# AY-Liu/Image-Editing-Framework

Hardware: AMD Instinct MI355X
Metric: denoising steps/sec (SD1.5 512x512 P2P edit step, UNet batch 4) (higher is better)
Workload: dtype f16x3; 1 GPU; sd15 UNet (859.5M params) P2P AttentionRefine edit step, 2 prompts x CFG = batch 4, 64x64 latents (512x512 px), 50-step DDIM, guidance 7.5, cross 0.8 / self 0.4, per-step null-text unconditional embeddings (P2P_NTI, edit_real.py); one independent edit per GPU; precision mode f16x3: fp32 storage; every contraction on split operands: hi + lo fp16 halves of each fp32 element, Ah Bh + Al Bh + Ah Bl =

## Files before the change

image-editing-framework_amd/csrc/exact_f32.hip:

```cpp
#include "ief_common.h"
#include "ief_params.h"
#include "x3_common.h"

#define XBM 128
#define XBK 32
#define XLD 36

__device__ __forceinline__ float silu_x(float x) { return x / (1.0f + expf(-x)); }

struct RowCoord { int b, oy, ox, ok; };

template <bool CONV, bool TRANSB, int NT>
__global__ __launch_bounds__(256) void igemm_f32_kernel(const IefGemmF32Params p) {
    constexpr int XBN = 64 * NT;
    __shared__ __attribute__((aligned(16))) float smem_x[2 * (XBM + XBN) * XLD];
    float* As = smem_x;
    float* Bs = smem_x + 2 * XBM * XLD;
    const int tid = threadIdx.x, lane = tid & 63, wid = tid >> 6;
    const int wm = wid >> 1, wn = wid & 1;
    const int li = lane & 31, lh = lane >> 5;
    const int ntn = (p.N + XBN - 1) / XBN;
    const int tm = blockIdx.x / ntn, tn = blockIdx.x - tm * ntn;
    const int m0 = tm * XBM, n0 = tn * XBN;
    const float* A = p.A;
// ... 875 lines not shown
static inline void gn3b_chunks(int HW, int C, int* nch, int* P) {
    const int CQ = C >> 2, CQB = CQ < 256 ? CQ : 256, PY = 256 / CQB;
    int p = GN3B_U * PY;
    if (p > HW) p = HW;
    *P = p;
    *nch = (HW + p - 1) / p;
}
extern "C" long long ief_groupnorm_bwd_f32_ws_floats(int B, int HW, int C) {
    int nch, P;
    gn3b_chunks(HW, C, &nch, &P);
    return ief_groupnorm_f32_ws_floats(B, HW, C) + 2ll * B * nch * C + 4ll * B * C;
}
__device__ __forceinline__ float dsilu_z(float z) {
    const float sg = 1.0f / (1.0f + expf(-z));
    return sg * (1.0f + z * (1.0f - sg));
}
template <int MODE>
__global__ __launch_bounds__(256) void gn3_bwd_kernel(const float* __restrict__ x, const float* __restrict__ x2, int C1, int C2,
                                                      const float* __restrict__ dy, const float* __restrict__ add, int HW, int P,
                                                      const float* __restrict__ gstats, const float* __restrict__ mom, int groups,
                                                      const float* __restrict__ gamma, const float* __restrict__ beta, int silu,
                                                      float* __restrict__ p1, float* __restrict__ p2, float* __restrict__ dx,
                                                      float* __restrict__ dx2) {
    __shared__ f32x4 red[256];
    const int C = C1 + C2, CQ = C >> 2, cpg = C / groups;
    const int CQB = CQ < 256 ? CQ : 256, PY = 256 / CQB;
    const int tid = threadIdx.x, cq = tid % CQB, py = tid / CQB;
    const bool lane_ok = py < PY;
    const int chunk = blockIdx.x, b = blockIdx.y, nch = gridDim.x;
    const int p0 = chunk * P, pn = min(P, HW - p0);
    for (int qb = 0; qb * CQB < CQ; ++qb) {
        const int q = qb * CQB + cq;
        const bool ok = lane_ok && q < CQ;
        const int c = ok ? q * 4 : 0;
        int cs = 4;
        const float* src = gn3_src(x, x2, C1, C2, b, HW, c, &cs) + (long long)p0 * cs;
        const float* dsrc = dy + ((long long)b * HW + p0) * C + c;
        f32x4 mu, rs, m1 = {0.f, 0.f, 0.f, 0.f}, m2 = {0.f, 0.f, 0.f, 0.f};
#pragma unroll
        for (int j = 0; j < 4; ++j) {
            const int g = (c + j) / cpg;
            mu[j] = gstats[((long long)b * groups + g) * 2];
            rs[j] = gstats[((long long)b * groups + g) * 2 + 1];
            if (MODE == 1) { m1[j] = mom[((long long)b * groups + g) * 2]; m2[j] = mom[((long long)b * groups + g) * 2 + 1]; }
        }
        const f32x4 ga = *(const f32x4*)(gamma + c), be = *(const f32x4*)(beta + c);
        f32x4 v[GN3B_U], d[GN3B_U];
#pragma unroll
        for (int u = 0; u < GN3B_U; ++u) {
            const int pp = py + u * PY;
            const bool in = ok && pp < pn;
            v[u] = in ? *(const f32x4*)(src + (long long)pp * cs) : f32x4{0.f, 0.f, 0.f, 0.f};
            d[u] = in ? *(const f32x4*)(dsrc + (long long)pp * C) : f32x4{0.f, 0.f, 0.f, 0.f};
        }
        f32x4 s1 = {0.f, 0.f, 0.f, 0.f}, s2 = {0.f, 0.f, 0.f, 0.f};
#pragma unroll
        for (int u = 0; u < GN3B_U; ++u) {
            const int pp = py + u * PY;
            if (!(ok && pp < pn)) continue;
            const f32x4 xh = (v[u] - mu) * rs;
            f32x4 gv = d[u] * ga;
            if (silu) {
#pragma unroll
                for (int j = 0; j < 4; ++j) gv[j] *= dsilu_z(xh[j] * ga[j] + be[j]);
            }
            if (MODE == 0) { s1 += gv; s2 += gv * xh; }
            else {
                f32x4 r = rs * (gv - m1 - xh * m2);
                if (add) r += *(const f32x4*)(add + ((long long)b * HW + p0 + pp) * C + c);
                float* dst = c < C1 ? dx + ((long long)b * HW + p0 + pp) * C1 + c : dx2 + ((long long)b * HW + p0 + pp) * C2 + (c - C1);
                *(f32x4*)dst = r;
            }
        }
        if (MODE == 0) {
            __syncthreads();
            red[tid] = s1;
            __syncthreads();
            f32x4 t1 = {0.f, 0.f, 0.f, 0.f};
            if (ok && py == 0) for (int y = 0; y < PY; ++y) t1 += red[y * CQB + cq];
            __syncthreads();
            red[tid] = s2;
            __syncthreads();
            if (ok && py == 0) {
                f32x4 t2 = {0.f, 0.f, 0.f, 0.f};
                for (int y = 0; y < PY; ++y) t2 += red[y * CQB + cq];
                const long long o = ((long long)b * nch + chunk) * C + c;
                *(f32x4*)(p1 + o) = t1;
                *(f32x4*)(p2 + o) = t2;
            }
        }
    }
}
__global__ __launch_bounds__(256) void gn3_bwd_finalize_kernel(const float* __restrict__ p1, const float* __restrict__ p2, int C, int HW,
                                                               int nch, int groups, float* __restrict__ mom) {
    __shared__ float sa[4], sb[4];
    const int b = blockIdx.x / groups, g = blockIdx.x - b * groups, cpg = C / groups, tid = threadIdx.x, lane = tid & 63;
    const int cl = tid % cpg, r0 = tid / cpg, rstep = 256 / cpg;
    float a = 0.f, q = 0.f;
    if (r0 < rstep) {
        const float* pa = p1 + (long long)b * nch * C + g * cpg + cl;
        const float* pq = p2 + (long long)b * nch * C + g * cpg + cl;
        for (int ch = r0; ch < nch; ch += rstep) { a += pa[(long long)ch * C]; q += pq[(long long)ch * C]; }
    }
#pragma unroll
    for (int off = 32; off > 0; off >>= 1) { a += __shfl_xor(a, off); q += __shfl_xor(q, off); }
    if (lane == 0) { sa[tid >> 6] = a; sb[tid >> 6] = q; }
    __syncthreads();
    if (tid == 0) {
        const float inv = 1.0f / ((float)HW * (float)cpg);
        mom[(long long)blockIdx.x * 2] = ((sa[0] + sa[1]) + (sa[2] + sa[3])) * inv;
        mom[(long long)blockIdx.x * 2 + 1] = ((sb[0] + sb[1]) + (sb[2] + sb[3])) * inv;
    }
}
extern "C" int ief_groupnorm_bwd_f32_ws(const float* x, const float* x2, int C1, int C2, const float* dy, const float* add, float* dx,
                                        float* dx2, const float* gamma, const float* beta, int B, int HW, int groups, float eps,
                                        int silu, float* ws, long long ws_floats, void* stream) {
    if (!x || !dy || !dx || !gamma || !beta || !ws || (C2 > 0 && (!x2 || !dx2))) return IEF_EINVAL;
    if (B <= 0 || HW <= 0 || groups <= 0 || C1 <= 0 || C2 < 0 || (C1 + C2) % groups || (C1 & 3) || (C2 & 3)) return IEF_ESHAPE;
    const int C = C1 + C2;
    if (C / groups > 256) return IEF_ESHAPE;
    if (ws_floats < ief_groupnorm_bwd_f32_ws_floats(B, HW, C)) return IEF_EINVAL;
    if (((uintptr_t)x | (uintptr_t)dy | (uintptr_t)dx | (uintptr_t)ws | (uintptr_t)(x2 ? x2 : x) | (uintptr_t)(dx2 ? dx2 : dx) |
         (uintptr_t)(add ? add : dy) | (uintptr_t)gamma | (uintptr_t)beta) & 15) return IEF_EALIGN;
    int nch, P, nchb, Pb;
    gn3_chunks(HW, C, &nch, &P);
    gn3b_chunks(HW, C, &nchb, &Pb);
    float* pmean = ws;
    float* pm2 = pmean + (long long)B * nch * C;
    float* scale = pm2 + (long long)B * nch * C;
    float* shift = scale + (long long)B * C;
    float* q1 = shift + (long long)B * C;
    float* q2 = q1 + (long long)B * nchb * C;
    float* gstats = q2 + (long long)B * nchb * C;
    float* mom = gstats + 2ll * B * groups;
    hipStream_t st = (hipStream_t)stream;
    hipLaunchKernelGGL(gn3_stats_kernel, dim3(nch, B), dim3(256), 0, st, x, x2, C1, C2, HW, P, pmean, pm2);
    IEF_LAUNCH_CHECK();
    hipLaunchKernelGGL(gn3_finalize_kernel, dim3(B * groups), dim3(256), 0, st, pmean, pm2, C, HW, P, nch, groups, eps, gamma, beta,
                       scale, shift, gstats);
    IEF_LAUNCH_CHECK();
    hipLaunchKernelGGL(gn3_bwd_kernel<0>, dim3(nchb, B), dim3(256), 0, st, x, x2, C1, C2, dy, add, HW, Pb, gstats, (const float*)nullptr,
                       groups, gamma, beta, silu, q1, q2, dx, dx2);
    IEF_LAUNCH_CHECK();
    hipLaunchKernelGGL(gn3_bwd_finalize_kernel, dim3(B * groups), dim3(256), 0, st, q1, q2, C, HW, nchb, groups, mom);
    IEF_LAUNCH_CHECK();
    hipLaunchKernelGGL(gn3_bwd_kernel<1>, dim3(nchb, B), dim3(256), 0, st, x, x2, C1, C2, dy, add, HW, Pb, gstats, mom, groups, gamma,
                       beta, silu, q1, q2, dx, dx2);
    IEF_LAUNCH_CHECK();
    return IEF_OK;
}

extern "C" int ief_groupnorm_silu_f32(const float* x, const float* x2, int C1, int C2, float* out, const float* gamma,
                                      const float* beta, int B, int HW, int groups, float eps, int silu, void* stream) {
    if (!x || !out || !gamma || !beta || (C2 > 0 && !x2)) return IEF_EINVAL;
    if (B <= 0 || HW <= 0 || groups <= 0 || C1 <= 0 || C2 < 0 || (C1 + C2) % groups) return IEF_ESHAPE;
    const int cpg = (C1 + C2) / groups;
    const bool al8 = (((uintptr_t)x | (uintptr_t)(x2 ? x2 : x) | (uintptr_t)out) & 7) == 0;
    if ((cpg & 1) || (C1 & 1) || (cpg >> 1) > 256 || !al8) {
        hipLaunchKernelGGL(groupnorm_f32_scalar_kernel, dim3(B * groups), dim3(256), 0, (hipStream_t)stream, x, x2, C1, C2, out,
                           gamma, beta, HW, groups, eps, silu);
        IEF_LAUNCH_CHECK();
        return IEF_OK;
    }
    const int cp2 = cpg >> 1;
    int PY = 512 / cp2;
    if (PY > HW) PY = HW;
    int threads = ((cp2 * PY + 63) / 64) * 64;
    if (threads > 512) { PY -= 1; threads = ((cp2 * PY + 63) / 64) * 64; }
    const int rounds = (HW + PY * 8 - 1) / (PY * 8);
    int KS = 1;
    while (KS * 2 <= rounds && B * groups * KS < 1024) KS *= 2;
    hipLaunchKernelGGL(groupnorm_f32_kernel, dim3(B * groups * KS), dim3(threads), 0, (hipStream_t)stream, x, x2, C1, C2, out,
                       gamma, beta, HW, groups, eps, silu, PY, KS);
    IEF_LAUNCH_CHECK();
    return IEF_OK;
}

extern "C" int ief_groupnorm_silu_x3p_small(const float* x, const float* x2, int C1, int C2, ief_half* outp, long long plane,
                                            const float* gamma, const float* beta, int B, int HW, int groups, float eps, int silu,
                                            void* stream) {
    if (!x || !outp || !gamma || !beta || (C2 > 0 && !x2)) return IEF_EINVAL;
    if (B <= 0 || HW <= 0 || groups <= 0 || C1 <= 0 || C2 < 0 || (C1 + C2) % groups || (plane & 1)) return IEF_ESHAPE;
    const int cpg = (C1 + C2) / groups;
    if ((cpg & 1) || (C1 & 1) || (cpg >> 1) > 256) return IEF_ESHAPE;
    if ((((uintptr_t)x | (uintptr_t)(x2 ? x2 : x)) & 7) || ((uintptr_t)outp & 3)) return IEF_EALIGN;
    const int cp2 = cpg >> 1;
    int PY = 512 / cp2;
    if (PY > HW) PY = HW;
    int threads = ((cp2 * PY + 63) / 64) * 64;
    if (threads > 512) { PY -= 1; threads = ((cp2 * PY + 63) / 64) * 64; }
    const int rounds = (HW + PY * 8 - 1) / (PY * 8);
    int KS = 1;
    while (KS * 2 <= rounds && B * groups * KS < 1024) KS *= 2;
    hipLaunchKernelGGL(groupnorm_f32_kernel, dim3(B * groups * KS), dim3(threads), 0, (hipStream_t)stream, x, x2, C1, C2, (float*)nullptr,
                       gamma, beta, HW, groups, eps, silu, PY, KS, (half_t*)outp, plane);
    IEF_LAUNCH_CHECK();
    return IEF_OK;
}

template <int E>
__global__ __launch_bounds__(1024) void groupnorm_reg_kernel(const float* __restrict__ x, const float* __restrict__ x2, int C1, int C2,
                                                             float* __restrict__ out, half_t* __restrict__ outp, long long plane,
                                                             const float* __restrict__ gamma, const float* __restrict__ beta, int HW,
                                                             int groups, float eps, int silu) {
    typedef __attribute__((ext_vector_type(2))) float f32x2;
    __shared__ float red[16];
    __shared__ float bc;
    __shared__ float sc_s[512], sh_s[512];
    const int C = C1 + C2, cpg = C / groups, cp2 = cpg >> 1;
    const int b = blockIdx.x / groups, g = blockIdx.x - b * groups;
    const int npairs = HW * cp2;
    const int tid = threadIdx.x;
    const int dq = 1024 / cp2, dr = 1024 - dq * cp2;
    int p = tid / cp2, j = tid - p * cp2;
    f32x2 v[E];
    const int p00 = p, j00 = j;
    const float* xb = x + (long long)b * HW * C1;
    const float* x2b = x2 ? x2 + (long long)b * HW * C2 : x;
#pragma unroll
    for (int k = 0; k < E; ++k) {
        const bool ok = tid + k * 1024 < npairs;
        const int c = g * cpg + (ok ? 2 * j : 0), pp = ok ? p : 0;
        const float* src = c < C1 ? xb + (unsigned)(pp * C1 + c) : x2b + (unsigned)(pp * C2 + (c - C1));
        const f32x2 t = *(const f32x2*)src;
        v[k] = ok ? t : (f32x2){0.f, 0.f};
        p += dq; j += dr;
        if (j >= cp2) { j -= cp2; ++p; }
        if ((k & 3) == 3) __builtin_amdgcn_sched_barrier(0);
    }
    auto block_sum = [&](float t) -> float {
        t = wave_sum(t);
        __syncthreads();
        if ((tid & 63) == 0) red[tid >> 6] = t;
        __syncthreads();
        if (tid == 0) { float a = 0.f; for (int w = 0; w < 16; ++w) a += red[w]; bc = a; }
        __syncthreads();
        return bc;
    };
    float s = 0.f;
#pragma unroll
    for (int k = 0; k < E; ++k) s += v[k][0] + v[k][1];
    const float n = (float)cpg * (float)HW;
    const float mean = block_sum(s) / n;
    float q = 0.f;
#pragma unroll
    for (int k = 0; k < E; ++k) {
        if (tid + k * 1024 < npairs) { const float d0 = v[k][0] - mean, d1 = v[k][1] - mean; q += d0 * d0 + d1 * d1; }
    }
    const float rstd = 1.0f / sqrtf(block_sum(q) / n + eps);
    if (tid < cpg) {
        const float sc = rstd * gamma[g * cpg + tid];
        sc_s[tid] = sc;
        sh_s[tid] = beta[g * cpg + tid] - mean * sc;
    }
    __syncthreads();
    p = p00; j = j00;
    float* ob = out ? out + (long long)b * HW * C : nullptr;
    half_t* opb = outp ? outp + (long long)b * HW * C : nullptr;
#pragma unroll
    for (int k = 0; k < E; ++k) {
        const int idx = tid + k * 1024;
        if (idx < npairs) {
            float y0 = v[k][0] * sc_s[2 * j] + sh_s[2 * j], y1 = v[k][1] * sc_s[2 * j + 1] + sh_s[2 * j + 1];
            if (silu) { y0 = silu_x(y0); y1 = silu_x(y1); }
            const unsigned o = (unsigned)(p * C + g * cpg + 2 * j);
            if (out) *(f32x2*)(ob + o) = (f32x2){y0, y1};
            if (outp) {
                const half2_t h = __builtin_convertvector((f32x2){y0, y1}, half2_t);
                const half2_t l = __builtin_convertvector((f32x2){y0 - (float)h[0], y1 - (float)h[1]}, half2_t);
                *(half2_t*)(opb + o) = h;
                *(half2_t*)(opb + plane + o) = l;
            }
        }
        p += dq; j += dr;
        if (j >= cp2) { j -= cp2; ++p; }
        if ((k & 3) == 3) __builtin_amdgcn_sched_barrier(0);
    }
}
extern "C" int ief_groupnorm_reg_fits(int C1, int C2, int HW, int groups) {
    if (groups <= 0 || C1 <= 0 || C2 < 0 || (C1 + C2) % groups) return 0;
    const int cpg = (C1 + C2) / groups;
    return !(cpg & 1) && !(C1 & 1) && cpg <= 512 && (long long)HW * cpg <= 40960;
}
extern "C" int ief_groupnorm_silu_reg(const float* x, const float* x2, int C1, int C2, float* out, ief_half* outp, long long plane,
                                      const float* gamma, const float* beta, int B, int HW, int groups, float eps, int silu,
                                      void* stream) {
    if (!x || (!out && !outp) || !gamma || !beta || (C2 > 0 && !x2)) return IEF_EINVAL;
    if (B <= 0 || HW <= 0 || !ief_groupnorm_reg_fits(C1, C2, HW, groups) || (plane & 1)) return IEF_ESHAPE;
    if ((((uintptr_t)x | (uintptr_t)(x2 ? x2 : x) | (uintptr_t)(out ? out : x)) & 7) || ((uintptr_t)outp & 3)) return IEF_EALIGN;
    const int cpg = (C1 + C2) / groups;
    const int need = (HW * (cpg >> 1) + 1023) / 1024;
    const dim3 grid(B * groups), blk(1024);
    hipStream_t st = (hipStream_t)stream;
#define GNR_GO(E_) hipLaunchKernelGGL(groupnorm_reg_kernel<E_>, grid, blk, 0, st, x, x2, C1, C2, out, (half_t*)outp, plane, gamma, beta, HW, groups, eps, silu)
    if (need <= 4) GNR_GO(4);
    else if (need <= 8) GNR_GO(8);
    else if (need <= 16) GNR_GO(16);
    else GNR_GO(20);
#undef GNR_GO
    IEF_LAUNCH_CHECK();
    return IEF_OK;
}

__global__ __launch_bounds__(256) void layernorm_f32_kernel(const float* __restrict__ x, float* __restrict__ out,
                                                            const float* __restrict__ gamma, const float* __restrict__ beta,
                                                            long long rows, int C, float eps) {
    const long long row = (long long)blockIdx.x * 4 + (threadIdx.x >> 6);
    if (row >= rows) return;
    const float* r = x + row * C;
    float* o = out + row * C;
    const int lane = threadIdx.x & 63;
    float s = 0.f;
    for (int i = lane; i < C; i += 64) s += r[i];
    const float mean = wave_sum(s) / (float)C;
    float q = 0.f;
    for (int i = lane; i < C; i += 64) { const float d = r[i] - mean; q += d * d; }
    const float rstd = 1.0f / sqrtf(wave_sum(q) / (float)C + eps);
    for (int i = lane; i < C; i += 64) o[i] = (r[i] - mean) * rstd * gamma[i] + beta[i];
}
template <int NV>
__global__ __launch_bounds__(256) void layernorm_f32_vec_kernel(const float* __restrict__ x, float* __restrict__ out,
                                                                const float* __restrict__ gamma, const float* __restrict__ beta,
                                                                long long rows, int C, float eps, half_t* __restrict__ outp = nullptr,
                                                                long long plane = 0) {
    const long long row = (long long)blockIdx.x * 4 + (threadIdx.x >> 6);
    if (row >= rows) return;
    const float* r = x + row * C;
    float* o = out + row * C;
    const int lane = threadIdx.x & 63, CQ = C >> 2;
    f32x4 v[NV];
    float s = 0.f;
#pragma unroll
    for (int j = 0; j < NV; ++j) {
        const int qd = lane + 64 * j;
        v[j] = qd < CQ ? *(const f32x4*)(r + qd * 4) : f32x4{0.f, 0.f, 0.f, 0.f};
        s += (v[j][0] + v[j][1]) + (v[j][2] + v[j][3]);
    }
    const float mean = wave_sum(s) / (float)C;
    float q = 0.f;
#pragma unroll
    for (int j = 0; j < NV; ++j) {
        if (lane + 64 * j < CQ) {
            const f32x4 d = v[j] - mean;
            q += (d[0] * d[0] + d[1] * d[1]) + (d[2] * d[2] + d[3] * d[3]);
        }
    }
    const float rstd = 1.0f / sqrtf(wave_sum(q) / (float)C + eps);
#pragma unroll
    for (int j = 0; j < NV; ++j) {
        const int qd = lane + 64 * j;
        if (qd < CQ) {
            const f32x4 y = (v[j] - mean) * rstd * *(const f32x4*)(gamma + qd * 4) + *(const f32x4*)(beta + qd * 4);
            if (out) *(f32x4*)(o + qd * 4) = y;
            if (outp) {
                half4 h, l;
                split4(y, 1.0f, h, l);
                half_t* op = outp + row * C + qd * 4;
                *(half4*)op = h;
                *(half4*)(op + plane) = l;
            }
        }
    }
}
extern "C" int ief_layernorm_x3p(const float* x, ief_half* outp, long long plane, const float* gamma, const float* beta, long long rows,
                                 int C, float eps, void* stream) {
    if (!x || !outp || !gamma || !beta) return IEF_EINVAL;
    if (rows <= 0 || C <= 0 || (C & 3) || C > 2560 || (plane & 3)) return IEF_ESHAPE;
    if ((((uintptr_t)x | (uintptr_t)gamma | (uintptr_t)beta) & 15) || ((uintptr_t)outp & 7)) return IEF_EALIGN;
    const dim3 grid((unsigned)((rows + 3) / 4));
    hipStream_t st = (hipStream_t)stream;
    float* none = nullptr;
    if (C <= 512) hipLaunchKernelGGL(layernorm_f32_vec_kernel<2>, grid, dim3(256), 0, st, x, none, gamma, beta, rows, C, eps, (half_t*)outp, plane);
    else if (C <= 1280) hipLaunchKernelGGL(layernorm_f32_vec_kernel<5>, grid, dim3(256), 0, st, x, none, gamma, beta, rows, C, eps, (half_t*)outp, plane);
    else hipLaunchKernelGGL(layernorm_f32_vec_kernel<10>, grid, dim3(256), 0, st, x, none, gamma, beta, rows, C, eps, (half_t*)outp, plane);
    IEF_LAUNCH_CHECK();
    return IEF_OK;
}
extern "C" int ief_layernorm_f32(const float* x, float* out, const float* gamma, const float* beta, long long rows, int C,
                                 float eps, void* stream) {
    if (!x || !out || !gamma || !beta) return IEF_EINVAL;
    if (rows <= 0 || C <= 0) return IEF_ESHAPE;
    const dim3 grid((unsigned)((rows + 3) / 4));
    hipStream_t st = (hipStream_t)stream;
    const bool vec = (C & 3) == 0 && ((((uintptr_t)x | (uintptr_t)out | (uintptr_t)gamma | (uintptr_t)beta) & 15) == 0);
    if (vec && C <= 512) hipLaunchKernelGGL(layernorm_f32_vec_kernel<2>, grid, dim3(256), 0, st, x, out, gamma, beta, rows, C, eps);
    else if (vec && C <= 1280) hipLaunchKernelGGL(layernorm_f32_vec_kernel<5>, grid, dim3(256), 0, st, x, out, gamma, beta, rows, C, eps);
    else if (vec && C <= 2560) hipLaunchKernelGGL(layernorm_f32_vec_kernel<10>, grid, dim3(256), 0, st, x, out, gamma, beta, rows, C, eps);
    else hipLaunchKernelGGL(layernorm_f32_kernel, grid, dim3(256), 0, st, x, out, gamma, beta, rows, C, eps);
    IEF_LAUNCH_CHECK();
    return IEF_OK;
}

__global__ __launch_bounds__(256) void ew_f32_kernel(const float* __restrict__ a, const float* __restrict__ b, float* __restrict__ out,
                                                     long long n, int which, int Ch) {
    for (long long i = (long long)blockIdx.x * 256 + threadIdx.x; i < n; i += (long long)gridDim.x * 256) {
        if (which == 0) out[i] = a[i] + b[i];
        else if (which == 1) out[i] = silu_x(a[i]);
        else {
            const long long row = i / Ch;
            const int c = (int)(i - row * Ch);
            const float* pr = a + row * 2 * Ch + (c >> 3) * 16 + (c & 7);
            out[i] = pr[0] * gelu_f(pr[8]);
        }
    }
}
__global__ __launch_bounds__(256) void geglu_il_f32_vec_kernel(const float* __restrict__ pre, float* __restrict__ out, long long nq, int Chq) {
    for (long long i = (long long)blockIdx.x * 256 + threadIdx.x; i < nq; i += (long long)gridDim.x * 256) {
        const long long row = i / Chq;
        const int cq = (int)(i - row * Chq);
        const float* pr = pre + row * (8ll * Chq) + (cq >> 1) * 16 + (cq & 1) * 4;
        const f32x4 hv = *(const f32x4*)pr, gv = *(const f32x4*)(pr + 8);
        f32x4 y;
#pragma unroll
        for (int j = 0; j < 4; ++j) y[j] = hv[j] * gelu_f(gv[j]);
        *(f32x4*)(out + i * 4) = y;
    }
}
static int launch_ew(const float* a, const float* b, float* out, long long n, int which, int Ch, void* stream) {
    if (!a || !out || (which == 0 && !b)) return IEF_EINVAL;
    if (n <= 0) return IEF_ESHAPE;
    int grid = (int)((n + 255) / 256);
    if (grid > 4096) grid = 4096;
    hipLaunchKernelGGL(ew_f32_kernel, dim3(grid), dim3(256), 0, (hipStream_t)stream, a, b, out, n, which, Ch);
    IEF_LAUNCH_CHECK();
    return IEF_OK;
}
extern "C" int ief_add_f32(const float* a, const float* b, float* out, long long n, void* stream) { return launch_ew(a, b, out, n, 0, 1, stream); }
extern "C" int ief_silu_f32(const float* x, float* out, long long n, void* stream) { return launch_ew(x, nullptr, out, n, 1, 1, stream); }
extern "C" int ief_geglu_il_f32(const float* pre, float* out, long long rows, int Ch, void* stream) {
    if (Ch <= 0 || (Ch & 7)) return IEF_ESHAPE;
    if (pre && out && rows > 0 && (((uintptr_t)pre | (uintptr_t)out) & 15) == 0) {
        const long long nq = rows * (Ch / 4);
        long long grid = (nq + 255) / 256;
        if (grid > 16384) grid = 16384;
        hipLaunchKernelGGL(geglu_il_f32_vec_kernel, dim3((unsigned)grid), dim3(256), 0, (hipStream_t)stream, pre, out, nq, Ch / 4);
        IEF_LAUNCH_CHECK();
        return IEF_OK;
    }
    return launch_ew(pre, nullptr, out, rows * Ch, 2, Ch, stream);
}

__global__ void timestep_embedding_f32_kernel(const float* __restrict__ t, float* __restrict__ out, int B, int dim) {
    const int half_dim = dim >> 1;
    const int i = blockIdx.x * blockDim.x + threadIdx.x;
    if (i >= B * half_dim) return;
    const int b = i / half_dim, k = i - b * half_dim;
    const float freq = expf(-9.210340371976184f * (float)k / (float)half_dim);
    const float a = t[b] * freq;
    out[(long long)b * dim + k] = cosf(a);
    out[(long long)b * dim + half_dim + k] = sinf(a);
}
extern "C" int ief_timestep_embedding_f32(const float* t, float* out, int B, int dim, void* stream) {
    if (!t || !out) return IEF_EINVAL;
    if (B <= 0 || dim <= 0 || (dim & 1)) return IEF_ESHAPE;
    const int n = B * (dim / 2);
    hipLaunchKernelGGL(timestep_embedding_f32_kernel, dim3((n + 255) / 256), dim3(256), 0, (hipStream_t)stream, t, out, B, dim);
    IEF_LAUNCH_CHECK();
    return IEF_OK;
}

__global__ __launch_bounds__(256) void gather_rows_f32_kernel(const f32x4* __restrict__ in, f32x4* __restrict__ out,
                                                              const int* __restrict__ src, int B, long long row4) {
    const long long total = (long long)B * row4;
    for (long long i = (long long)blockIdx.x * 256 + threadIdx.x; i < total; i += (long long)gridDim.x * 256) {
        const int b = (int)(i / row4);
        out[i] = in[(long long)src[b] * row4 + (i - (long long)b * row4)];
    }
}
extern "C" int ief_gather_rows_f32(const float* in, float* out, const int* src, int B, long long row_elems, void* stream) {
    if (!in || !out || !src) return IEF_EINVAL;
    if (B <= 0 || row_elems <= 0 || (row_elems & 3)) return IEF_ESHAPE;
    if (((uintptr_t)in | (uintptr_t)out) & 15) return IEF_EALIGN;
    const long long total = (long long)B * (row_elems / 4);
    int grid = (int)((total + 255) / 256);
    if (grid > 2048) grid = 2048;
    hipLaunchKernelGGL(gather_rows_f32_kernel, dim3(grid), dim3(256), 0, (hipStream_t)stream, (const f32x4*)in, (f32x4*)out, src,
                       B, row_elems / 4);
    IEF_LAUNCH_CHECK();
    return IEF_OK;
}

template <int CIN, bool PL = false>
__global__ __launch_bounds__(256) void conv_in_f32_kernel(const float* __restrict__ x, const float* __restrict__ w,
                                                          const float* __restrict__ bias, float* __restrict__ out, int B, int Cin,
                                                          int H, int Wd, int Cout, half_t* __restrict__ outp = nullptr,
                                                          long long plane = 0) {
    const int C4 = Cout >> 2;
    const long long total = (long long)B * H * Wd * C4;
    for (long long i = (long long)blockIdx.x * 256 + threadIdx.x; i < total; i += (long long)gridDim.x * 256) {
        const long long pix = i / C4;
        const int c4 = (int)(i - pix * C4);
        const int b = (int)(pix / (H * Wd));
        const int rem = (int)(pix - (long long)b * H * Wd);
        const int oy = rem / Wd, ox = rem - oy * Wd;
        f32x4 acc = {0.f, 0.f, 0.f, 0.f};
        if constexpr (CIN > 0) {
#pragma unroll
            for (int ky = 0; ky < 3; ++ky) {
                const int iy = oy + ky - 1;
                const bool yok = (unsigned)iy < (unsigned)H;
                float v[3][CIN];
                f32x4 wv[3][CIN];
#pragma unroll
                for (int kx = 0; kx < 3; ++kx) {
                    const int ix = ox + kx - 1;
                    const bool ok = yok && (unsigned)ix < (unsigned)Wd;
#pragma unroll
                    for (int ci = 0; ci < CIN; ++ci) {
                        v[kx][ci] = ok ? x[(((long long)b * CIN + ci) * H + iy) * Wd + ix] : 0.f;
                        wv[kx][ci] = *(const f32x4*)(w + ((long long)((ky * 3 + kx) * CIN + ci)) * Cout + c4 * 4);
                    }
                }
#pragma unroll
                for (int kx = 0; kx < 3; ++kx) {
                    const int ix = ox + kx - 1;
                    if (!(yok && (unsigned)ix < (unsigned)Wd)) continue;
#pragma unroll
                    for (int ci = 0; ci < CIN; ++ci)
#pragma unroll
                        for (int e = 0; e < 4; ++e) acc[e] += v[kx][ci] * wv[kx][ci][e];
                }
            }
        } else {
            for (int tap = 0; tap < 9; ++tap) {
                const int iy = oy + tap / 3 - 1, ix = ox + tap % 3 - 1;
                if ((unsigned)iy >= (unsigned)H || (unsigned)ix >= (unsigned)Wd) continue;
                for (int ci = 0; ci < Cin; ++ci) {
                    const float v = x[(((long long)b * Cin + ci) * H + iy) * Wd + ix];
                    const f32x4 wv = *(const f32x4*)(w + ((long long)(tap * Cin + ci)) * Cout + c4 * 4);
#pragma unroll
                    for (int e = 0; e < 4; ++e) acc[e] += v * wv[e];
                }
            }
        }
        if (bias) {
#pragma unroll
            for (int e = 0; e < 4; ++e) acc[e] += bias[c4 * 4 + e];
        }
        *(f32x4*)(out + pix * Cout + c4 * 4) = acc;
        if constexpr (PL) {
            half4 hh, ll;
            split4(acc, 1.0f, hh, ll);
            half_t* op = outp + pix * Cout + c4 * 4;
            *(half4*)op = hh;
            *(half4*)(op + plane) = ll;
        }
    }
}
extern "C" int ief_conv_in_f32act(const float* x, const float* w, const float* bias, float* out, int B, int Cin, int H, int Wd,
                                  int Cout, void* stream) {
    if (!x || !w || !out) return IEF_EINVAL;
    if (B <= 0 || H <= 0 || Wd <= 0 || Cin <= 0 || Cin > 8 || Cout <= 0 || (Cout & 3)) return IEF_ESHAPE;
    if (((uintptr_t)w | (uintptr_t)out) & 15) return IEF_EALIGN;
    const long long total = (long long)B * H * Wd * (Cout / 4);
    int grid = (int)((total + 255) / 256);
    if (grid > 8192) grid = 8192;
    if (Cin == 4) hipLaunchKernelGGL((conv_in_f32_kernel<4, false>), dim3(grid), dim3(256), 0, (hipStream_t)stream, x, w, bias, out, B, Cin, H, Wd, Cout, (half_t*)nullptr, 0ll);
    else hipLaunchKernelGGL((conv_in_f32_kernel<0, false>), dim3(grid), dim3(256), 0, (hipStream_t)stream, x, w, bias, out, B, Cin, H, Wd, Cout, (half_t*)nullptr, 0ll);
    IEF_LAUNCH_CHECK();
    return IEF_OK;
}

extern "C" int ief_conv_in_f32act_planes(const float* x, const float* w, const float* bias, float* out, ief_half* outp, long long plane,
                                         int B, int Cin, int H, int Wd, int Cout, void* stream) {
    if (!x || !w || !out || !outp) return IEF_EINVAL;
    if (B <= 0 || H <= 0 || Wd <= 0 || Cin <= 0 || Cin > 8 || Cout <= 0 || (Cout & 3) || plane <= 0 || (plane & 3)) return IEF_ESHAPE;
    if ((((uintptr_t)w | (uintptr_t)out) & 15) || ((uintptr_t)outp & 7)) return IEF_EALIGN;
    const long long total = (long long)B * H * Wd * (Cout / 4);
    int grid = (int)((total + 255) / 256);
    if (grid > 8192) grid = 8192;
    if (Cin == 4) hipLaunchKernelGGL((conv_in_f32_kernel<4, true>), dim3(grid), dim3(256), 0, (hipStream_t)stream, x, w, bias, out, B, Cin, H, Wd, Cout, (half_t*)outp, plane);
    else hipLaunchKernelGGL((conv_in_f32_kernel<0, true>), dim3(grid), dim3(256), 0, (hipStream_t)stream, x, w, bias, out, B, Cin, H, Wd, Cout, (half_t*)outp, plane);
    IEF_LAUNCH_CHECK();
    return IEF_OK;
}

__global__ __launch_bounds__(256) void conv_out_f32_kernel(const float* __restrict__ x, const float* __restrict__ w,
                                                           const float* __restrict__ bias, float* __restrict__ out, int B, int C,
                                                           int H, int Wd, int Cout) {
    const int sub = threadIdx.x & 15;
    const long long pix = (long long)blockIdx.x * 16 + (threadIdx.x >> 4);
    const long long total = (long long)B * H * Wd;
    const bool live = pix < total;
    const long long pc = live ? pix : 0;
    const int b = (int)(pc / (H * Wd));
    const int rem = (int)(pc - (long long)b * H * Wd);
    const int oy = rem / Wd, ox = rem - oy * Wd;
    const int C4 = C >> 2;
    float acc[8];
#pragma unroll
    for (int o = 0; o < 8; ++o) acc[o] = 0.f;
    if (live) {
        for (int tap = 0; tap < 9; ++tap) {
            const int ky = tap / 3, kx = tap - ky * 3;
            const int iy = oy + ky - 1, ix = ox + kx - 1;
            if ((unsigned)iy >= (unsigned)H || (unsigned)ix >= (unsigned)Wd) continue;
            const float* xp = x + (((long long)b * H + iy) * Wd + ix) * C;
            for (int c4 = sub; c4 < C4; c4 += 16) {
                const f32x4 v = *(const f32x4*)(xp + c4 * 4);
#pragma unroll
                for (int o = 0; o < 8; ++o) {
                    if (o < Cout) {
                        const f32x4 wv = *(const f32x4*)(w + ((long long)o * 9 + tap) * C + c4 * 4);
#pragma unroll
                        for (int e = 0; e < 4; ++e) acc[o] += v[e] * wv[e];
                    }
                }
            }
        }
    }
#pragma unroll
    for (int o = 0; o < 8; ++o) {
#pragma unroll
        for (int off = 8; off > 0; off >>= 1) acc[o] += __shfl_xor(acc[o], off);
    }
    if (live && sub == 0) {
        for (int o = 0; o < Cout; ++o) out[(((long long)b * Cout + o) * H + oy) * Wd + ox] = acc[o] + (bias ? bias[o] : 0.f);
    }
}
template <int CH>
__global__ __launch_bounds__(256) void conv_out_f32_lds_kernel(const float* __restrict__ x, const float* __restrict__ w,
                                                               const float* __restrict__ bias, float* __restrict__ out, int B, int C,
                                                               int H, int Wd, int Cout) {
    extern __shared__ __attribute__((aligned(16))) float wl_f32[];
    const int sub = threadIdx.x & 15;
    const long long pix = (long long)blockIdx.x * 16 + (threadIdx.x >> 4);
    const long long total = (long long)B * H * Wd;
    const bool live = pix < total;
    const long long pc = live ? pix : 0;
    const int b = (int)(pc / (H * Wd));
    const int rem = (int)(pc - (long long)b * H * Wd);
    const int oy = rem / Wd, ox = rem - oy * Wd;
    const int C4 = C >> 2;
    const int nw4 = (Cout * 9 * C) >> 2;
    for (int i = threadIdx.x; i < nw4; i += 256) ((f32x4*)wl_f32)[i] = ((const f32x4*)w)[i];
    __syncthreads();
    float acc[8];
#pragma unroll
    for (int o = 0; o < 8; ++o) acc[o] = 0.f;
#pragma unroll
    for (int ky = 0; ky < 3; ++ky) {
        const int iy = oy + ky - 1;
        const bool yok = live && (unsigned)iy < (unsigned)H;
        f32x4 v[3][CH];
#pragma unroll
        for (int kx = 0; kx < 3; ++kx) {
            const int ix = ox + kx - 1;
            const bool ok = yok && (unsigned)ix < (unsigned)Wd;
            const float* xp = x + (((long long)b * H + (ok ? iy : 0)) * Wd + (ok ? ix : 0)) * C;
#pragma unroll
            for (int j = 0; j < CH; ++j) {
                const int c4 = sub + 16 * j;
                v[kx][j] = (ok && c4 < C4) ? *(const f32x4*)(xp + c4 * 4) : f32x4{0.f, 0.f, 0.f, 0.f};
            }
        }
#pragma unroll
        for (int kx = 0; kx < 3; ++kx) {
            const int ix = ox + kx - 1;
            if (!(yok && (unsigned)ix < (unsigned)Wd)) continue;
            const int tap = ky * 3 + kx;
#pragma unroll
            for (int j = 0; j < CH; ++j) {
                const int c4 = sub + 16 * j;
                if (c4 < C4) {
#pragma unroll
                    for (int o = 0; o < 8; ++o) {
                        if (o < Cout) {
                            const f32x4 wv = *(const f32x4*)(wl_f32 + (o * 9 + tap) * C + c4 * 4);
#pragma unroll
                            for (int e = 0; e < 4; ++e) acc[o] += v[kx][j][e] * wv[e];
                        }
                    }
                }
            }
        }
    }
#pragma unroll
// ... 50 lines not shown
```

image-editing-framework_amd/csrc/gemm_x3p.hip:

```cpp
#include "ief_common.h"
#include "ief_params.h"
#include "x3_common.h"

#include "x3p_common.h"

template <int BM, int BN, int WAVES_M, int WAVES_N, int NS, int NL, bool CONV>
__global__ __launch_bounds__(64 * (WAVES_M * WAVES_N + NL)) void igemm_x3p_kernel(const IefGemmX3pParams p) {
    constexpr int BK = XP_BK;
    constexpr int NWC = WAVES_M * WAVES_N;
    constexpr int NSW = NL > 0 ? NL : NWC;
    constexpr int PA = BM / 16, PB = BN / 16;
    constexpr int P = 2 * (PA + PB);
    constexpr int G = (P + NSW - 1) / NSW;
    constexpr int WM = BM / WAVES_M, WN = BN / WAVES_N, TM = WM / 16, TN = WN / 16;
    constexpr int SLOT = P * 16 * BK;
    constexpr int DUMP = NS * SLOT;
    static_assert(BM % 16 == 0 && BN % 16 == 0 && WM % 16 == 0 && WN % 16 == 0, "tile");
    static_assert(NS >= 2 && NS <= 4, "ring depth");
    static_assert((NS * SLOT + 512) * 2 <= 160 * 1024, "LDS");
    __shared__ __attribute__((aligned(1024))) half_t smem[NS * SLOT + 512];

    const int tid = threadIdx.x, lane = tid & 63;
    const int wave = __builtin_amdgcn_readfirstlane(tid >> 6);
    const int wr = wave / WAVES_N, wc = wave % WAVES_N;
// ... 139 lines not shown
    }
    const int fr = lane & 15, fq = lane >> 4;
    int aoff[TM], boff[TN];
#pragma unroll
    for (int i = 0; i < TM; ++i) {
        const int row = wr * WM + i * 16 + fr;
        aoff[i] = row * BK + ((fq ^ xp_swz(row)) << 3);
    }
#pragma unroll
    for (int j = 0; j < TN; ++j) {
        const int row = wc * WN + j * 16 + fr;
        boff[j] = 2 * BM * BK + row * BK + ((fq ^ xp_swz(row)) << 3);
    }
    half8 ah[TM], al[TM], bh[TN], bl[TN];
    auto read_frags = [&](const half_t* S) {
#pragma unroll
        for (int i = 0; i < TM; ++i) { ah[i] = *(const half8*)(S + aoff[i]); al[i] = *(const half8*)(S + aoff[i] + BM * BK); }
#pragma unroll
        for (int j = 0; j < TN; ++j) { bh[j] = *(const half8*)(S + boff[j]); bl[j] = *(const half8*)(S + boff[j] + BN * BK); }
    };
    auto mfma_frags = [&]() {
#pragma unroll
        for (int j = 0; j < TN; ++j)
#pragma unroll
            for (int i = 0; i < TM; ++i) {
                acc[j][i] = __builtin_amdgcn_mfma_f32_16x16x32_f16(bl[j], ah[i], acc[j][i], 0, 0, 0);
                acc[j][i] = __builtin_amdgcn_mfma_f32_16x16x32_f16(bh[j], al[i], acc[j][i], 0, 0, 0);
                acc[j][i] = __builtin_amdgcn_mfma_f32_16x16x32_f16(bh[j], ah[i], acc[j][i], 0, 0, 0);
            }
    };
    auto read_mfma_wide = [&](const half_t* S) {
#pragma unroll
        for (int i = 0; i < TM; ++i) { ah[i] = *(const half8*)(S + aoff[i]); al[i] = *(const half8*)(S + aoff[i] + BM * BK); }
#pragma unroll
        for (int j = 0; j < TN; ++j) {
            const half8 wh = *(const half8*)(S + boff[j]), wl = *(const half8*)(S + boff[j] + BN * BK);
#pragma unroll
            for (int i = 0; i < TM; ++i) {
                acc[j][i] = __builtin_amdgcn_mfma_f32_16x16x32_f16(wl, ah[i], acc[j][i], 0, 0, 0);
                acc[j][i] = __builtin_amdgcn_mfma_f32_16x16x32_f16(wh, al[i], acc[j][i], 0, 0, 0);
                acc[j][i] = __builtin_amdgcn_mfma_f32_16x16x32_f16(wh, ah[i], acc[j][i], 0, 0, 0);
            }
        }
    };
    constexpr bool PINGPONG = NWC == 8 && NS >= 3;
    const bool late = PINGPONG && wave >= 4 && wave < NWC;
#pragma unroll
    for (int s = 0; s < NS - 1; ++s)
        if (kt_lo + s < nk) stage_tile(s);
    if (NL > 0 && !computes) {
        for (int kt = kt_lo; kt < nk; kt += NS) {
#pragma unroll
            for (int s = 0; s < NS; ++s) {
                const int k = kt + s;
                if (k < nk) {
                    if (nk - 1 - k >= NS - 2) asm volatile("s_waitcnt vmcnt(%0)" ::"n"(G * (NS - 2)) : "memory");
                    else asm volatile("s_waitcnt vmcnt(0)" ::: "memory");
                    XP_BARRIER();
                    if (k + NS - 1 < nk) stage_tile((s + NS - 1) % NS);
                }
            }
        }
    } else if (!late) {
        for (int kt = kt_lo; kt < nk; kt += NS) {
#pragma unroll
            for (int s = 0; s < NS; ++s) {
                const int k = kt + s;
                if (k < nk) {
                    if constexpr (NL == 0) {
                        if (nk - 1 - k >= NS - 2) asm volatile("s_waitcnt vmcnt(%0)" ::"n"(G * (NS - 2)) : "memory");
                        else asm volatile("s_waitcnt vmcnt(0)" ::: "memory");
                    }
                    XP_BARRIER();
                    if constexpr (NL == 0) { if (k + NS - 1 < nk) stage_tile((s + NS - 1) % NS); }
                    if constexpr (TN > 5) {
                        read_mfma_wide(smem + s * SLOT);
                    } else {
                        read_frags(smem + s * SLOT);
                        mfma_frags();
                    }
                }
            }
        }
    } else {
        for (int kt = kt_lo; kt < nk; kt += NS) {
#pragma unroll
            for (int s = 0; s < NS; ++s) {
                const int k = kt + s;
                if (k < nk) {
                    if constexpr (NL == 0) {
                        if (nk - 1 - k >= NS - 2) asm volatile("s_waitcnt vmcnt(%0) lgkmcnt(0)" ::"n"(G * (NS - 2)) : "memory");
                        else asm volatile("s_waitcnt vmcnt(0) lgkmcnt(0)" ::: "memory");
                    } else {
                        asm volatile("s_waitcnt lgkmcnt(0)" ::: "memory");
                    }
                    XP_BARRIER();
                    if (k > kt_lo) mfma_frags();
                    if constexpr (NL == 0) { if (k + NS - 1 < nk) stage_tile((s + NS - 1) % NS); }
                    read_frags(smem + s * SLOT);
                }
            }
        }
        if (nk > kt_lo) mfma_frags();
    }
    if (!computes) return;

    constexpr int NP2 = TN / 2;
    const int cb = n0 + wc * WN;
    const float inv = p.inv_scale;
    if (p.splits > 1) {
        float* slab = p.ws + (long long)blockIdx.y * p.M * p.N;
#pragma unroll
        for (int i = 0; i < TM; ++i) {
            const int m = m0 + wr * WM + i * 16 + fr;
            if (m >= p.M) continue;
#pragma unroll
            for (int j = 0; j < TN; ++j) {
                const int n = j < 2 * NP2 ? cb + 32 * (j >> 1) + 8 * fq + 4 * (j & 1) : cb + j * 16 + 4 * fq;
                if (n < p.N) *(f32x4*)(slab + (long long)m * p.N + n) = acc[j][i] * inv;
            }
        }
        return;
    }
    if (p.geglu) {
#pragma unroll
        for (int i = 0; i < TM; ++i) {
            const int m = m0 + wr * WM + i * 16 + fr;
            float mu = 0.f, rs = 1.f;
            if (p.rstat_in && m < p.M) xp_ln_row(p, m, mu, rs);
#pragma unroll
            for (int P = 0; P < NP2; ++P) {
                const int nh = cb + 32 * P + 16 * (fq >> 1) + 4 * (fq & 1), ng = nh + 8;
                if (m >= p.M || nh >= p.N) continue;
                f32x4 hv = acc[2 * P][i] * inv, gv = acc[2 * P + 1][i] * inv;
                if (p.rstat_in) {
                    hv = (hv - *(const f32x4*)(p.colsum + nh) * mu) * rs;
                    gv = (gv - *(const f32x4*)(p.colsum + ng) * mu) * rs;
                }
                if (p.bias) { hv += *(const f32x4*)(p.bias + nh); gv += *(const f32x4*)(p.bias + ng); }
                f32x4 o;
#pragma unroll
                for (int e = 0; e < 4; ++e) o[e] = hv[e] * gelu_nb(gv[e]) * p.out_scale;
                const int no = cb / 2 + 16 * P + 4 * fq;
                if (p.Out) *(f32x4*)(p.Out + (long long)m * p.ldo + no) = o;
                if (p.OutP) {
                    half4 h, l;
                    split4(o, 1.0f, h, l);
                    half_t* op = p.OutP + (long long)m * p.ldp + no;
                    *(half4*)op = h;
                    *(half4*)(op + p.planeO) = l;
                }
            }
            if constexpr (TN & 1) {
                constexpr int j = TN - 1;
                const int nb = cb + j * 16, n = nb + 4 * fq;
                const bool lo_half = fq < 2;
                f32x4 v = acc[j][i] * inv;
                if (p.rstat_in && n < p.N) v = (v - *(const f32x4*)(p.colsum + n) * mu) * rs;
                if (p.bias && n < p.N) v += *(const f32x4*)(p.bias + n);
                const float x0 = __shfl_xor(lo_half ? v[2] : v[0], 32), x1 = __shfl_xor(lo_half ? v[3] : v[1], 32);
                const float o0 = (lo_half ? v[0] * gelu_nb(x0) : x0 * gelu_nb(v[2])) * p.out_scale;
                const float o1 = (lo_half ? v[1] * gelu_nb(x1) : x1 * gelu_nb(v[3])) * p.out_scale;
                const int no = nb / 2 + (lo_half ? 4 * fq : 4 * (fq - 2) + 2);
                if (m < p.M && nb < p.N) {
                    if (p.Out) *(f32x2*)(p.Out + (long long)m * p.ldo + no) = f32x2{o0, o1};
                    if (p.OutP) {
                        const half2_t h = __builtin_convertvector(f32x2{o0, o1}, half2_t);
                        float r0, r1;
                        asm("v_fma_mix_f32 %0, %1, 1.0, -%2 op_sel:[0,0,0] op_sel_hi:[0,0,1]" : "=v"(r0) : "v"(o0), "v"(h));
                        asm("v_fma_mix_f32 %0, %1, 1.0, -%2 op_sel:[0,0,1] op_sel_hi:[0,0,1]" : "=v"(r1) : "v"(o1), "v"(h));
                        half_t* op = p.OutP + (long long)m * p.ldp + no;
                        *(half2_t*)op = h;
                        *(half2_t*)(op + p.planeO) = __builtin_convertvector(f32x2{r0, r1}, half2_t);
                    }
                }
            }
        }
        return;
    }
    const int slots_out = (p.N + WN - 1) / WN;
#pragma unroll
    for (int i = 0; i < TM; ++i) {
        const int m = m0 + wr * WM + i * 16 + fr;
        const bool mok = m < p.M;
        float mu = 0.f, rs = 1.f;
        if (p.rstat_in && mok) xp_ln_row(p, m, mu, rs);
        f32x4 vv[TN];
#pragma unroll
        for (int j = 0; j < TN; ++j) vv[j] = f32x4{0.f, 0.f, 0.f, 0.f};
#pragma unroll
        for (int P = 0; P < NP2; ++P) {
            const int n = cb + 32 * P + 8 * fq;
            if (!mok || n >= p.N) continue;
            f32x4 v0 = acc[2 * P][i] * inv, v1 = acc[2 * P + 1][i] * inv;
            if (n + 4 < p.N) {
                if (p.rstat_in) {
                    v0 = (v0 - *(const f32x4*)(p.colsum + n) * mu) * rs;
                    v1 = (v1 - *(const f32x4*)(p.colsum + n + 4) * mu) * rs;
                }
                xp_store8(p, v0, v1, m, n);
                vv[2 * P] = v0; vv[2 * P + 1] = v1;
            } else {
                if (p.rstat_in) v0 = (v0 - *(const f32x4*)(p.colsum + n) * mu) * rs;
                vv[2 * P] = xp_store(p, v0, m, n);
            }
        }
        if constexpr (TN & 1) {
            constexpr int j = TN - 1;
            const int n = cb + j * 16 + 4 * fq;
            if (mok && n < p.N) {
                f32x4 v = acc[j][i] * inv;
                if (p.rstat_in) v = (v - *(const f32x4*)(p.colsum + n) * mu) * rs;
                vv[j] = xp_store(p, v, m, n);
            }
        }
        if (p.rstat_out) {
            float sm, sq;
            xp_row_stats<TN>(vv, sm, sq);
            if (fq == 0 && mok && cb < p.N) {
                float* ro = p.rstat_out + ((long long)m * slots_out + cb / WN) * 2;
                ro[0] = sm; ro[1] = sq;
            }
        }
    }
}

__global__ __launch_bounds__(256) void x3p_reduce_kernel(const IefGemmX3pParams p) {
    const int N4 = p.N >> 2;
    const long long total = (long long)p.M * N4, slab = (long long)p.M * p.N;
    for (long long i = (long long)blockIdx.x * 256 + threadIdx.x; i < total; i += (long long)gridDim.x * 256) {
        const int m = (int)(i / N4), n = (int)(i - (long long)m * N4) * 4;
        const float* w = p.ws + (long long)m * p.N + n;
        f32x4 a = *(const f32x4*)w;
        int s = 1;
        for (; s + 3 < p.splits; s += 4) {
            f32x4 t[4];
#pragma unroll
            for (int u = 0; u < 4; ++u) t[u] = *(const f32x4*)(w + (s + u) * slab);
#pragma unroll
            for (int u = 0; u < 4; ++u) a += t[u];
        }
        for (; s < p.splits; ++s) a += *(const f32x4*)(w + s * slab);
        xp_store(p, a, m, n);
    }
}

__global__ __launch_bounds__(256) void x3_split_act_kernel(const float* __restrict__ x, half_t* __restrict__ planes, long long plane,
                                                           long long rows, int C4, int ldx, int ldp, float scale) {
    const long long total = rows * C4;
    for (long long i = (long long)blockIdx.x * 256 + threadIdx.x; i < total; i += (long long)gridDim.x * 256) {
        const long long r = i / C4;
        const int c = (int)(i - r * C4) * 4;
        half4 h, l;
        split4(*(const f32x4*)(x + r * ldx + c), scale, h, l);
        half_t* o = planes + r * ldp + c;
        *(half4*)o = h;
        *(half4*)(o + plane) = l;
    }
}
extern "C" int ief_x3_split_act(const float* x, ief_half* planes, long long plane, long long rows, int C, int ldx, int ldp, float scale,
                                void* stream) {
    if (!x || !planes) return IEF_EINVAL;
    if (rows <= 0 || C <= 0 || (C & 3) || (ldx & 3) || (ldp & 3) || (plane & 3) || !(scale > 0.f)) return IEF_ESHAPE;
    if (((uintptr_t)x & 15) || ((uintptr_t)planes & 7)) return IEF_EALIGN;
    long long grid = (rows * (C / 4) + 255) / 256;
    if (grid > 16384) grid = 16384;
    hipLaunchKernelGGL(x3_split_act_kernel, dim3((unsigned)grid), dim3(256), 0, (hipStream_t)stream, x, (half_t*)planes, plane, rows,
                       C / 4, ldx, ldp, scale);
    IEF_LAUNCH_CHECK();
    return IEF_OK;
}

extern "C" int ief_gemm_x3p_tile_bm(int tile) {
    switch (tile) {
        case 1: case 2: case 3: case 7: return 128;
        case 4: case 8: case 11: case 12: case 13: return 256;
        case 5: return 64;
        case 6: return 128;
        default: return 0;
    }
}
extern "C" int ief_gemm_x3p_tile_wn(int tile) { return tile == 6 ? 64 : tile == 8 ? 160 : 80; }
extern "C" int ief_gemm_x3p_tile_bn(int tile) {
    switch (tile) {
        case 1: case 2: case 4: case 5: case 7: return 160;
        case 3: case 11: case 12: case 13: return 80;
        case 6: return 64;
        case 8: return 320;
        default: return 0;
    }
}

template <int BM, int BN, int WAVES_M, int WAVES_N, int NS, int NL>
static int launch_x3p(const IefGemmX3pParams& p, hipStream_t st) {
    const int tiles = ((p.M + BM - 1) / BM) * ((p.N + BN - 1) / BN);
    const int splits = p.splits > 1 ? p.splits : 1;
    constexpr int NT = 64 * (WAVES_M * WAVES_N + NL);
    if (p.conv) hipLaunchKernelGGL((igemm_x3p_kernel<BM, BN, WAVES_M, WAVES_N, NS, NL, true>), dim3(tiles, splits), dim3(NT), 0, st, p);
    else hipLaunchKernelGGL((igemm_x3p_kernel<BM, BN, WAVES_M, WAVES_N, NS, NL, false>), dim3(tiles, splits), dim3(NT), 0, st, p);
    IEF_LAUNCH_CHECK();
    return IEF_OK;
}

int ief_conv_halo_x3p_dispatch(const IefGemmX3pParams& p, hipStream_t st);

extern "C" int ief_gemm_x3p(const IefGemmX3pParams* pp, void* stream) {
    if (!pp || !pp->A || !pp->W || !pp->zeros || (!pp->Out && !pp->OutP)) return IEF_EINVAL;
    IefGemmX3pParams p = *pp;
    if (p.M <= 0 || p.N <= 0 || p.K <= 0 || (p.K % XP_BK) || (p.N & 3)) return IEF_ESHAPE;
    if (p.rowvec && p.rows_per_batch <= 0) return IEF_ESHAPE;
    if (p.splits > 1 && (!p.ws || p.splits > 64 || p.geglu || p.rstat_out || p.cstat_out)) return IEF_EINVAL;
    if (!(p.inv_scale > 0.f)) return IEF_EINVAL;
    if ((p.ldw & 7) || (p.planeW & 7) || ((uintptr_t)p.W & 15)) return IEF_EALIGN;
    if (p.Out && ((p.ldo & 3) || ((uintptr_t)p.Out & 15))) return IEF_EALIGN;
    if (p.OutP && ((p.ldp & 3) || (p.planeO & 3) || ((uintptr_t)p.OutP & 7))) return IEF_EALIGN;
    if ((p.bias && ((uintptr_t)p.bias & 15)) || (p.rowvec && ((uintptr_t)p.rowvec & 15)) ||
        (p.residual && (((uintptr_t)p.residual & 15) || (p.ldr & 3)))) return IEF_EALIGN;
    if (p.geglu && ((p.N & 15) || p.residual || p.rowvec)) return IEF_EINVAL;
    if (p.rstat_out && (p.splits > 1 || p.geglu || p.tile == 11 || p.tile == 12 || p.tile == 13 || (p.N % ief_gemm_x3p_tile_wn(p.tile)))) return IEF_EINVAL;
    if (p.rstat_in && (!p.colsum || p.rstat_slots <= 0 || p.rstat_cnt <= 0 || p.rstat_slots * p.rstat_cnt != p.K || p.splits > 1 ||
                       p.conv || !(p.ln_eps > 0.f) || ((uintptr_t)p.colsum & 15))) return IEF_EINVAL;
    if (p.conv) {
        if (p.C1 <= 0 || p.C2 < 0 || (p.C1 % XP_BK) || (p.C2 % XP_BK) || (p.CE1 % XP_BK) || (p.CE2 % XP_BK)) return IEF_ESHAPE;
        if ((p.C2 > 0 && !p.A2) || (p.CE1 > 0 && !p.E1) || (p.CE2 > 0 && !p.E2) || (p.CE2 > 0 && p.CE1 == 0)) return IEF_EINVAL;
        if (p.stride != 1 && p.stride != 2) return IEF_ESHAPE;
        if (p.ups != 0 && p.ups != 1) return IEF_ESHAPE;
        if (p.ups && ((p.H | p.Wd) & 1)) return IEF_ESHAPE;
        if ((p.CE1 + p.CE2) > 0 && (p.stride != 1 || p.ups)) return IEF_ESHAPE;
        const int ktaps = p.tile == 13 ? 4 : 9;
        if (p.K != ktaps * (p.C1 + p.C2) + p.CE1 + p.CE2 || p.batch_images <= 0 || p.M != p.batch_images * p.Ho * p.Wo) return IEF_ESHAPE;
        const long long in_pix = (long long)p.batch_images * (p.H >> p.ups) * (p.Wd >> p.ups);
        const int cmax = p.C1 > p.C2 ? p.C1 : p.C2, emax = p.CE1 > p.CE2 ? p.CE1 : p.CE2;
        if (in_pix * cmax * 2 >= (1ll << 32) || (long long)p.M * emax * 2 >= (1ll << 32)) return IEF_ESHAPE;
        if (((uintptr_t)p.A & 15) || (p.planeA & 7) || (p.A2 && (((uintptr_t)p.A2 & 15) || (p.planeA2 & 7))) ||
            (p.E1 && (((uintptr_t)p.E1 & 15) || (p.planeE1 & 7))) || (p.E2 && (((uintptr_t)p.E2 & 15) || (p.planeE2 & 7)))) return IEF_EALIGN;
    } else {
        if ((p.lda & 7) || (p.planeA & 7) || ((uintptr_t)p.A & 15)) return IEF_EALIGN;
    }
    hipStream_t st = (hipStream_t)stream;
    int rc;
    switch (p.tile) {
        case 2: rc = launch_x3p<128, 160, 4, 2, 4, 4>(p, st); break;
        case 3: rc = launch_x3p<128, 80, 4, 1, 3, 0>(p, st); break;
        case 4: rc = launch_x3p<256, 160, 4, 2, 3, 0>(p, st); break;
        case 5: rc = launch_x3p<64, 160, 2, 2, 4, 0>(p, st); break;
        case 6: rc = launch_x3p<128, 64, 4, 1, 3, 0>(p, st); break;
        case 7: rc = launch_x3p<128, 160, 2, 2, 2, 0>(p, st); break;
        case 8: rc = launch_x3p<256, 320, 4, 2, 2, 0>(p, st); break;
        case 11: case 12: case 13: rc = ief_conv_halo_x3p_dispatch(p, st); break;
        case 1: default: rc = launch_x3p<128, 160, 4, 2, 4, 0>(p, st); break;
    }
    if (rc) return rc;
    if (p.splits > 1) {
        const long long total = (long long)p.M * (p.N / 4);
        int grid = (int)((total + 255) / 256);
        if (grid > 8192) grid = 8192;
        hipLaunchKernelGGL(x3p_reduce_kernel, dim3(grid), dim3(256), 0, st, p);
        IEF_LAUNCH_CHECK();
    }
    return IEF_OK;
}
```

image-editing-framework_amd/planes.py:

```python
import os
from ctypes import byref

import torch

from . import hip
from .hip import IefGemmX3pParams, _check, _dev32, _ptr, _shape, _stream, _Timed, _zeros

ACT_SCALE = 1.0
W_SCALE = hip.X3_SCALE_W


class Planes:
    __slots__ = ("t",)

    def __init__(self, t):
        if not (isinstance(t, torch.Tensor) and t.dtype == torch.float16 and t.dim() >= 2 and t.shape[0] == 2 and t.stride(-1) == 1):
            raise TypeError("Planes: expected an fp16 tensor [2, ...] with a contiguous last dimension")
        if not t.is_cuda:
            raise TypeError("Planes: device tensor expected (no CPU path)")
        self.t = t

    @staticmethod
    def empty(*shape, device):
        return Planes(torch.empty(2, *shape, dtype=torch.float16, device=device))

    @property
    def shape(self):
        return self.t.shape[1:]

    @property
    def device(self):
        return self.t.device

    @property
    def hi(self):
        return self.t[0]

    @property
    def lo(self):
        return self.t[1]

    @property
    def plane(self):
        return self.t.stride(0)

    def dim(self):
        return self.t.dim() - 1

    def __getitem__(self, idx):
        if not isinstance(idx, tuple):
            idx = (idx,)
        return Planes(self.t[(slice(None),) + idx])

    def reshape(self, *shape):
        return Planes(self.t.reshape(2, *shape))

    def is_contiguous(self):
        return self.t[0].is_contiguous()

    def to_f32(self):
        return self.t[0].float() + self.t[1].float()

    def rows_ld(self, name="planes"):
        h = self.t[0]
        cols = h.shape[-1]
        ld = h.stride(-2) if h.dim() >= 2 else cols
        rows = 1
        for s in h.shape[:-1]:
            rows *= s
        for d in range(h.dim() - 2):
            if h.shape[d] > 1 and h.stride(d) != h.stride(d + 1) * h.shape[d + 1]:
                raise ValueError(f"{name}: leading dimensions must collapse to rows of one stride")
        return rows, cols, ld


def split(x, out=None, scale=ACT_SCALE):
    lib = hip.load()
    rows, C, ldx = hip._rows_ld32(x, "x")
    if out is None:
        out = Planes.empty(*x.shape, device=x.device)
    _, _, ldp = out.rows_ld("out")
    with _Timed("x3_split_act_kernel", 0.0, 8.0 * rows * C):
        _check(lib.ief_x3_split_act(x.data_ptr(), out.t.data_ptr(), out.plane, rows, C, ldx, ldp, float(scale), _stream()), "ief_x3_split_act")
    return out


def weight_planes(w):
    t = hip.x3_weight_planes(w, W_SCALE)
    if t is None:
        raise RuntimeError("weight planes missing while capturing: run one eager forward first")
    return t


_PLAN_FILE = os.environ.get("IEF_PLAN_FILE_X3") or os.path.join(os.path.dirname(os.path.abspath(__file__)), "tuned_plans_x3.json")
_plans = None
TILE_FORCE = int(os.environ.get("IEF_X3P_TILE", "0"))


def _plan_table():
    global _plans
    if _plans is None:
        _plans = hip.read_plans(_PLAN_FILE)
    return _plans


def save_plans(path=None):
    hip.write_plans(path or _PLAN_FILE, _plan_table())


_TILES = {1: (128, 160), 2: (128, 160), 3: (128, 80), 4: (256, 160), 5: (64, 160), 6: (128, 64), 7: (128, 160), 8: (256, 320),
          11: (256, 80), 12: (256, 80), 13: (256, 80)}
_HALO = (11, 12, 13)


def heuristic_plan(M, N, K, conv=False):
    nk = K // 32
    if N % 80 and N % 64 == 0:
        tile = 6
    elif N % 160:
        tile = 3
    elif M <= 64:
        tile = 5
    else:
        t1 = -(-M // 128) * (N // 160)
        tile = 4 if t1 >= 1024 and M % 256 == 0 else 1
    bm, bn = _TILES[tile]
    tiles = -(-M // bm) * -(-N // bn)
    splits = 1
    if tiles < 160 and nk >= 16:
        splits = max(1, min(-(-256 // tiles), nk // 8, 16))
    return tile, splits


def halo_fallback_plan(M, N, ncb):
    tiles = -(-M // 256) * (N // 80)
    sp = 1
    while tiles * sp < 192 and sp * 2 <= ncb // 2 and sp < 16:
        sp *= 2
    return 11, sp


def pick_plan(M, N, K, conv=False, variant=""):
    hit = _plan_table().get(f"{'conv' if conv else 'gemm'}|{M}|{N}|{K}{variant}")
    if hit is None:
        hit = heuristic_plan(M, N, K, conv)
    if TILE_FORCE and (TILE_FORCE < 10 or conv):
        return TILE_FORCE, hit[1]
    return hit[0], hit[1]


AUTOTUNE = os.environ.get("IEF_AUTOTUNE_X3", "0") == "1"


def candidate_plans(M, N, K, conv=False, halo_ok=False, ncb=0, geglu=False, phase_ok=False):
    nk = K // 32
    out = []
    for t, (bm, bn) in _TILES.items():
        if t in _HALO:
            continue
        if N % bn or (t == 6 and N % 80 == 0):
            continue
        tiles = -(-M // bm) * (N // bn)
        for sp in (1, 2, 3, 4, 6, 8, 12, 16):
            if sp > 1 and (geglu or nk // sp < 4 or tiles * sp > 2048 or tiles >= 512):
                continue
            if tiles * sp < 40 and sp < 16:
                continue
            out.append((t, sp))
    if conv and halo_ok:
        tiles = -(-M // 256) * (N // 80)
        for sp in (1, 2, 3, 4, 5, 6, 8, 10, 12, 16, 20):
            if sp > 1 and (sp > ncb // 2 or tiles * sp > 1024 or tiles >= 384):
                continue
            if tiles * sp < 40 and sp < 16:
                continue
            out.append((11, sp))
    if conv and phase_ok:
        tiles = -(-(M // 4) // 256) * (N // 80) * 4
        for sp in (1, 2, 3, 4, 5, 6, 8, 10, 12, 16, 20):
            if sp > 1 and (sp > ncb // 2 or tiles * sp > 1024 or tiles >= 384):
                continue
            if tiles * sp < 40 and sp < 16:
                continue
            out.append((13, sp))
    return out


def _autotune(key, cands, run, w):
    wc = hip._cold_copies(w)
    for x in wc:
        weight_planes(x)
        if any(t == 13 for t, _ in cands):
            hip.x3_upsample_phase_planes(x, W_SCALE)
    best = None
    for t, sp in cands:
        try:
            us = hip._time_graph(lambda i: run(t, sp, wc[i % len(wc)]))
        except (RuntimeError, ValueError):
            continue
        if best is None or us < best[0]:
            best = (us, t, sp)
    for x in wc[1:]:
        hip._x3_planes.pop((x.data_ptr(), tuple(x.shape), float(W_SCALE)), None)
        hip._x3_planes.pop((x.data_ptr(), tuple(x.shape), float(W_SCALE), "phase"), None)
    if best is not None:
        _plan_table()[key] = (best[1], best[2])
    return best


def supported(N, K):
    return (N % 80 == 0 or N % 64 == 0) and K % 32 == 0


def _out_args(p, M, No, out, out_planes, device, lead_shape):
    o32 = op = None
    if out is True or isinstance(out, torch.Tensor) or (out is None and out_planes in (None, False)):
        o32 = out if isinstance(out, torch.Tensor) else torch.empty(*lead_shape, No, dtype=torch.float32, device=device)
        Mo, Nn, ldo = hip._rows_ld32(o32, "out")
        if (Mo, Nn) != (M, No):
            raise ValueError("x3p: out shape mismatch")
        p.Out, p.ldo = o32.data_ptr(), ldo
    if out_planes not in (None, False):
        op = out_planes if isinstance(out_planes, Planes) else Planes.empty(*lead_shape, No, device=device)
        Mp, Np, ldp = op.rows_ld("out_planes")
        if (Mp, Np) != (M, No):
            raise ValueError("x3p: out_planes shape mismatch")
        p.OutP, p.planeO, p.ldp = op.t.data_ptr(), op.plane, ldp
    return o32, op


def _ret(o32, op):
    if o32 is not None and op is not None:
        return o32, op
    return o32 if op is None else op


class RowStats:
    __slots__ = ("buf", "slots", "cnt")

    def __init__(self, buf, slots, cnt):
        self.buf, self.slots, self.cnt = buf, slots, cnt


class FoldedLN:
    __slots__ = ("w", "bias", "colsum", "eps")

    def __init__(self, w, bias, gamma, beta, eps):
        wf = (w * gamma[None, :]).contiguous()
        self.w = wf
        b = w @ beta
        self.bias = (b if bias is None else b + bias).contiguous()
        pl = weight_planes(wf)
        self.colsum = ((pl[0].float().sum(1) + pl[1].float().sum(1)) / W_SCALE).contiguous()
        self.eps = eps


LN_FOLD = os.environ.get("IEF_X3P_FOLD_LN", "0") == "1"


def gemm(a, w, bias=None, residual=None, rowvec=None, rows_per_batch=0, out=None, out_planes=None, out_scale=1.0,
         geglu=False, tile=0, splits=0, row_stats=False, ln=None):
    lib = hip.load()
    if not isinstance(a, Planes):
        raise TypeError("planes.gemm: a must be Planes")
    M, K, lda = a.rows_ld("a")
    N = w.shape[0]
    if w.dim() != 2 or w.shape[1] != K:
        raise ValueError(f"planes.gemm: K mismatch {tuple(w.shape)} vs {K}")
    wp = weight_planes(w)
    p = IefGemmX3pParams()
    p.A, p.planeA, p.lda = a.t.data_ptr(), a.plane, lda
    p.W, p.planeW, p.ldw = wp.data_ptr(), wp.stride(0), K
    No = N // 2 if geglu else N
    o32, op = _out_args(p, M, No, out, out_planes, a.device, a.shape[:-1])
    p.M, p.N, p.K = M, N, K
    p.out_scale, p.inv_scale = out_scale, 1.0 / (ACT_SCALE * W_SCALE)
    p.geglu, p.zeros = 1 if geglu else 0, _zeros(a.device)
    if tile:
        p.tile, p.splits = tile, max(1, splits)
    else:
        key = f"gemm|{M}|{N}|{K}" + ("|g" if geglu else "")
        if AUTOTUNE and key not in _plan_table() and not hip._capturing() and hip._prof is None:
            _autotune(key, candidate_plans(M, N, K, geglu=geglu),
                      lambda t, sp, wi: gemm(a, wi, bias=bias, residual=residual, rowvec=rowvec, rows_per_batch=rows_per_batch, out=out,
                                             out_planes=out_planes, out_scale=out_scale, geglu=geglu, tile=t, splits=sp), w)
        p.tile, p.splits = pick_plan(M, N, K, variant="|g" if geglu else "")
    if geglu or row_stats or ln is not None:
        p.splits = 1
    rs = None
    if row_stats:
        wn = lib.ief_gemm_x3p_tile_wn(p.tile)
        if N % wn:
            raise ValueError("planes.gemm: row statistics need N to be a multiple of the tile's wave width")
        rs = RowStats(torch.empty(M, N // wn, 2, dtype=torch.float32, device=a.device), N // wn, wn)
        p.rstat_out = rs.buf.data_ptr()
    if ln is not None:
        st, colsum, eps = ln
        if st.buf.shape[0] != M or st.slots * st.cnt != K or _dev32(colsum, "colsum").numel() != N:
            raise ValueError("planes.gemm: ln statistics / colsum do not match this launch")
        p.rstat_in, p.rstat_slots, p.rstat_cnt, p.colsum, p.ln_eps = st.buf.data_ptr(), st.slots, st.cnt, colsum.data_ptr(), eps
    ws = hip._fill_epilogue(p, hip._rows_ld32, "planes.gemm", M, N, a.device, bias, rowvec, rows_per_batch, residual, p.splits)
    nbytes = 4.0 * (M * K + N * K + M * No * ((1 if o32 is not None else 0) + (1 if op is not None else 0)) + (M * N if residual is not None else 0))
    kn = f"igemm_x3p_kernel<false> t{p.tile}" + (f" {M}x{N}x{K} s{p.splits}" if hip.PROF_SHAPES else "")
    bm, bn = _TILES[p.tile]
    hip.note_staged(kn, 4.0 * K * (bm + bn) * -(-M // bm) * -(-N // bn))
    with _Timed(kn, 2.0 * M * N * K, nbytes):
        _check(lib.ief_gemm_x3p(byref(p), _stream()), "ief_gemm_x3p")
    r = _ret(o32, op)
    if row_stats:
        return (r + (rs,)) if isinstance(r, tuple) else (r, rs)
    return r


def conv3x3(x, w, bias=None, x2=None, stride=1, upsample=False, rowvec=None, residual=None, out=None, out_planes=None,
            extra=None, pad_hi_only=False, tile=0, splits=0):
    lib = hip.load()
    if not isinstance(x, Planes) or (x2 is not None and not isinstance(x2, Planes)):
        raise TypeError("planes.conv3x3: x / x2 must be Planes")
    if not x.is_contiguous() or (x2 is not None and not x2.is_contiguous()) or not w.is_contiguous():
        raise ValueError("planes.conv3x3: x, x2, w must be contiguous")
    e1, e2 = (None, None) if extra is None else extra
    for e in (e1, e2):
        if e is not None and (not isinstance(e, Planes) or not e.is_contiguous()):
            raise ValueError("planes.conv3x3: extra sources must be contiguous NHWC Planes at the output resolution")
    if residual is not None and not hip._act32(residual, "residual").is_contiguous():
        raise ValueError("planes.conv3x3: residual must be contiguous fp32 [B, Ho, Wo, Cout]")
    g = hip.conv_geometry(x.shape, w.shape, hip._shape(x2), None if extra is None else (e1.shape, hip._shape(e2)), hip._shape(rowvec),
                          hip._shape(residual), stride, upsample, pad_hi_only, "planes.conv3x3")
    B, Hp, Wp, C1, C2, CE1, CE2, Cout, H, Wd, Ho, Wo, M, K = g[:14]
    p = IefGemmX3pParams()
    p.A, p.planeA = x.t.data_ptr(), x.plane
    if x2 is not None:
        p.A2, p.planeA2 = x2.t.data_ptr(), x2.plane
    if e1 is not None:
        p.E1, p.planeE1 = e1.t.data_ptr(), e1.plane
    if e2 is not None:
        p.E2, p.planeE2 = e2.t.data_ptr(), e2.plane
    o32, op = _out_args(p, M, Cout, out, out_planes, x.device, (B, Ho, Wo))
    p.M, p.N, p.K = M, Cout, K
    p.conv, p.H, p.Wd, p.C1, p.C2, p.Ho, p.Wo = 1, H, Wd, C1, C2, Ho, Wo
    p.stride, p.ups, p.batch_images, p.pad_hi_only = stride, 1 if upsample else 0, B, 1 if pad_hi_only else 0
    p.CE1, p.CE2 = CE1, CE2
    p.out_scale, p.inv_scale, p.zeros = 1.0, 1.0 / (ACT_SCALE * W_SCALE), _zeros(x.device)
    halo_ok = HALO and g.halo_geom and Cout % 80 == 0
    phase_ok = HALO and g.phase_geom and Cout % 80 == 0
    if tile:
        p.tile, p.splits = tile, max(1, splits)
    else:
        variant = ("|u" if upsample else "") + (f"|s{stride}" if stride != 1 else "") + ("|e" if extra is not None else "")
        key = f"conv|{M}|{Cout}|{K}{variant}"
        if AUTOTUNE and key not in _plan_table() and not hip._capturing() and hip._prof is None:
            _autotune(key, candidate_plans(M, Cout, K, conv=True, halo_ok=halo_ok, ncb=(C1 + C2) // 32, phase_ok=phase_ok),
                      lambda t, sp, wi: conv3x3(x, wi, bias, x2=x2, stride=stride, upsample=upsample, rowvec=rowvec, residual=residual,
                                                out=out, out_planes=out_planes, extra=extra, pad_hi_only=pad_hi_only, tile=t, splits=sp), w)
        hit = _plan_table().get(key)
        if hit is not None and (hit[0] not in _HALO or (phase_ok if hit[0] == 13 else halo_ok)):
            p.tile, p.splits = hit[0], hit[1]
        elif halo_ok:
            p.tile, p.splits = halo_fallback_plan(M, Cout, (C1 + C2) // 32)
        else:
            p.tile, p.splits = heuristic_plan(M, Cout, K, conv=True)
            if TILE_FORCE and TILE_FORCE < 10:
                p.tile = TILE_FORCE
    if p.tile == 13:
        if not phase_ok:
            raise ValueError("planes.conv3x3: this geometry has no phase form (tile 13)")
        p.splits = min(p.splits, (C1 + C2) // 32)
        wp = hip.x3_upsample_phase_planes(w, W_SCALE)
        if wp is None:
            raise RuntimeError("phase weight planes missing while capturing: run one eager forward first")
        K = 4 * (C1 + C2)
        p.K = K
    else:
        if p.tile in (11, 12):
            if not halo_ok:
                raise ValueError("planes.conv3x3: this geometry has no halo form (tile 11 / 12)")
            p.tile = 12 if upsample else 11
            p.splits = min(p.splits, (C1 + C2) // 32)
        wp = weight_planes(w)
    p.W, p.planeW, p.ldw = wp.data_ptr(), wp.stride(0), K
    ws = hip._fill_epilogue(p, hip._rows_ld32, "planes.conv3x3", M, Cout, x.device, bias, rowvec, g.rows_per_batch, residual, p.splits)
    nbytes = 4.0 * (B * Hp * Wp * (C1 + C2) + M * (CE1 + CE2) + Cout * K + M * Cout * ((1 if o32 is not None else 0) + (1 if op is not None else 0) + (1 if residual is not None else 0)))
    kn = "conv3x3_halo_x3p_kernel_phase" if p.tile == 13 else \
        f"conv3x3_halo_x3p_kernel<{'true' if upsample else 'false'}>" if p.tile in (11, 12) else f"igemm_x3p_kernel<true> t{p.tile}"
    kn += f" {M}x{Cout}x{K} s{p.splits}" if hip.PROF_SHAPES else ""
    if p.tile == 13:
        hip.note_staged(kn, 4.0 * (C1 + C2) * (4 * 80 + 256 + 2 * (Wp + 1)) * -(-(M // 4) // 256) * -(-Cout // 80) * 4)
    elif p.tile in (11, 12):
        hip.note_staged(kn, 4.0 * (C1 + C2) * (9 * 80 + 256 + 2 * (Wd + 1)) * -(-M // 256) * -(-Cout // 80))
    else:
        bm, bn = _TILES[p.tile]
        hip.note_staged(kn, 4.0 * K * (bm + bn) * -(-M // bm) * -(-Cout // bn))
    with _Timed(kn, 2.0 * M * Cout * K, nbytes):
        _check(lib.ief_gemm_x3p(byref(p), _stream()), "ief_gemm_x3p (conv)")
    return _ret(o32, op)


GN_SMALL_ELEMS = int(os.environ.get("IEF_GN_SMALL_ELEMS", str(3 << 20)))
GN_REG_MAX_HW = int(os.environ.get("IEF_GN_REG_MAX_HW", "1024"))
HALO = os.environ.get("IEF_X3P_HALO", "1") == "1"
ENABLED = os.environ.get("IEF_X3P", "1") == "1"


def groupnorm(x, gamma, beta, groups, eps, silu=False, x2=None, out32=False):
    lib = hip.load()
    if not hip._act32(x, "x").is_contiguous() or (x2 is not None and not hip._act32(x2, "x2").is_contiguous()):
        raise ValueError("planes.groupnorm: inputs must be contiguous")
    B, C1 = x.shape[0], x.shape[-1]
    C2 = 0 if x2 is None else x2.shape[-1]
    HW = x.numel() // (B * C1)
    out = Planes.empty(*x.shape[:-1], C1 + C2, device=x.device)
    cpg = (C1 + C2) // groups
    if HW <= GN_REG_MAX_HW and lib.ief_groupnorm_reg_fits(C1, C2, HW, groups):
        o32 = torch.empty(*x.shape[:-1], C1 + C2, dtype=torch.float32, device=x.device) if out32 else None
        with _Timed("groupnorm_reg_kernel", 0.0, (12.0 if out32 else 8.0) * (x.numel() + (0 if x2 is None else x2.numel()))):
            _check(lib.ief_groupnorm_silu_reg(x.data_ptr(), _ptr(x2), C1, C2, _ptr(o32), out.t.data_ptr(), out.plane,
                                              _dev32(gamma, "gamma").data_ptr(), _dev32(beta, "beta").data_ptr(), B, HW, groups,
                                              eps, 1 if silu else 0, _stream()), "ief_groupnorm_silu_reg")
        return (out, o32) if out32 else out
    if not out32 and HW <= GN_REG_MAX_HW and B * HW * (C1 + C2) <= GN_SMALL_ELEMS and cpg % 2 == 0 and C1 % 2 == 0 and cpg // 2 <= 256:
        with _Timed("groupnorm_f32_kernel", 0.0, 12.0 * (x.numel() + (0 if x2 is None else x2.numel()))):
            _check(lib.ief_groupnorm_silu_x3p_small(x.data_ptr(), _ptr(x2), C1, C2, out.t.data_ptr(), out.plane,
                                                    _dev32(gamma, "gamma").data_ptr(), _dev32(beta, "beta").data_ptr(), B, HW, groups,
                                                    eps, 1 if silu else 0, _stream()), "ief_groupnorm_silu_x3p_small")
        return out
    o32 = torch.empty(*x.shape[:-1], C1 + C2, dtype=torch.float32, device=x.device) if out32 else None
    nws = lib.ief_groupnorm_f32_ws_floats(B, HW, C1 + C2)
    ws = torch.empty(nws, dtype=torch.float32, device=x.device)
    with _Timed("gn3_f32 (stats + finalize + apply)", 0.0, 12.0 * (x.numel() + (0 if x2 is None else x2.numel()))):
        _check(lib.ief_groupnorm_silu_x3p_ws(x.data_ptr(), _ptr(x2), C1, C2, _ptr(o32), out.t.data_ptr(), out.plane,
                                             _dev32(gamma, "gamma").data_ptr(), _dev32(beta, "beta").data_ptr(), B, HW, groups, eps,
                                             1 if silu else 0, ws.data_ptr(), nws, _stream()), "ief_groupnorm_silu_x3p_ws")
    return (out, o32) if out32 else out


def layernorm(x, gamma, beta, eps=1e-5):
    lib = hip.load()
    if not hip._act32(x, "x").is_contiguous():
        raise ValueError("planes.layernorm: x must be contiguous")
    C = x.shape[-1]
    out = Planes.empty(*x.shape, device=x.device)
    with _Timed("layernorm_f32_vec_kernel", 0.0, 8.0 * x.numel()):
        _check(lib.ief_layernorm_x3p(x.data_ptr(), out.t.data_ptr(), out.plane, _dev32(gamma, "gamma").data_ptr(),
                                     _dev32(beta, "beta").data_ptr(), x.numel() // C, C, eps, _stream()), "ief_layernorm_x3p")
    return out


def attn_out_args(p, B, N, C, device, out32=False):
    op = Planes.empty(B, N, C, device=device)
    p.OutP, p.planeO, p.sOPb, p.ldp = op.t.data_ptr(), op.plane, N * C, C
    o32 = None
    if out32:
        o32 = torch.empty(B, N, C, dtype=torch.float32, device=device)
        p.Out, p.sOb, p.ldo = o32.data_ptr(), N * C, C
    return op, o32


def _hi(t, name):
    if not isinstance(t, Planes) or t.dim() != 3:
        raise TypeError(f"planes.attn_flash: {name} must be Planes [B, rows, heads*d]")
    return t.hi


FLASH_PLANES = os.environ.get("IEF_X3P_FLASH", "1") == "1"
FLASH_PLANES_DIMS = (40, 64, 80)


KEY_SPLIT_MAX = 8
KEY_SPLIT_MIN_TILES = 8
KEY_SPLIT_SETTINGS = (1, 2, 4, 8, "auto")


def key_split_setting(v):
    if isinstance(v, str):
        v = v.strip().lower()
        if v == "auto":
            return "auto"
        v = int(v)
    v = int(v)
    if v < 1:
        raise ValueError(f"attn_key_splits must be >= 1 or 'auto', got {v}")
    return v


def _flash_key_tile(d):
    return 64 if d == 40 else 32


def attn_key_splits(B, heads, N, L, d, cus=None, setting="auto") -> int:
    setting = key_split_setting(setting)
    if d not in FLASH_PLANES_DIMS or L < 1:
        return 1
    nt = -(-L // _flash_key_tile(d))
    if setting != "auto":
        T = -(-nt // min(setting, nt))
        return -(-nt // T)
    if L < 128:
        return 1
    if cus is None:
        cus = torch.cuda.get_device_properties(torch.cuda.current_device()).multi_processor_count
    G = -(-N // (256 if d == 40 else 128)) * B * heads
    S = KEY_SPLIT_MAX if 2 * G <= cus else 1
    while S > 1 and (G * S > 2 * cus or nt // S < KEY_SPLIT_MIN_TILES):
        S //= 2
    if S <= 1:
        return 1
    T = -(-nt // S)
    return -(-nt // T)


def attn_flash(q, k, v, heads, scale, q_src=None, k_src=None, v_src=None, out=None, out_planes=True, lse=None, key_splits=1,
               q_idx=None, k_idx=None, gate=None, q_cls=None, k_cls=None, k2_src=None, v2_src=None):
    lib = hip.load()
    idx = q_idx is not None or k_idx is not None
    cls = q_cls is not None or k_cls is not None
    uni = k2_src is not None or v2_src is not None
    if uni and (k2_src is None or v2_src is None):
        raise ValueError("planes.attn_flash: k2_src and v2_src go together")
    if uni and (idx or cls or lse is not None or key_splits != 1):
        raise ValueError("planes.attn_flash: a two-segment launch (k2_src / v2_src) takes no lists and no class words, writes no "
                         "lse and does not split its keys")
    if idx and (q_idx is None or k_idx is None):
        raise ValueError("planes.attn_flash: q_idx and k_idx go together")
    if cls and (q_cls is None or k_cls is None):
        raise ValueError("planes.attn_flash: q_cls and k_cls go together")
    if cls and (idx or lse is not None or key_splits != 1):
        raise ValueError("planes.attn_flash: a class-masked launch (q_cls / k_cls) takes no lists, writes no lse and does not "
                         "split its keys")
    if gate is not None and not (idx or cls):
        raise ValueError("planes.attn_flash: gate needs q_idx / k_idx or q_cls / k_cls")
    if idx and (lse is not None or key_splits != 1):
        raise ValueError("planes.attn_flash: a gathered launch (q_idx / k_idx) writes no lse and does not split its keys")
    dest_p = out_planes if isinstance(out_planes, Planes) else None
    if idx and dest_p is None and out is None:
        raise ValueError("planes.attn_flash: with q_idx / k_idx only the listed rows are written: pass the existing destination "
                         "as out= (fp32) or out_planes= (Planes)")
    if cls and dest_p is None and out is None:
        raise ValueError("planes.attn_flash: a class-masked launch overwrites rows of an existing destination: pass it as out= "
                         "(fp32) or out_planes= (Planes)")
    if dest_p is not None and not (idx or cls):
        raise ValueError("planes.attn_flash: out_planes=<Planes> is the destination of a gathered launch (q_idx / k_idx) or a "
                         "class-masked one (q_cls / k_cls)")
    for t, nm in ((q, "q"), (k, "k"), (v, "v")):
        hip._attn_layout(t, nm, _hi)
    dest = (dest_p if dest_p is not None else out) if idx or cls else None
    if dest_p is not None and out is not None and hip._act32(out, "out").shape != dest_p.shape:
        raise ValueError("planes.attn_flash: out and out_planes must have one shape")
    g = hip.attn_geometry(_shape(q), _shape(k), _shape(v), heads, out=_shape(dest), lse=_shape(lse), q_src=q_src is not None,
                          k_src=k_src is not None, v_src=v_src is not None, batch=None if dest is None else dest.shape[0],
                          who="planes.attn_flash")
    B, N, L, C, d = g
    if d not in FLASH_PLANES_DIMS:
        raise ValueError(f"planes.attn_flash: head dim {d} has no planes instantiation")
    for t, nm in ((q_src, "q_src"), (k_src, "k_src"), (v_src, "v_src")):
        if dest is not None and t is not None and t.numel() != B:
            raise ValueError(f"planes.attn_flash: {nm} must have one entry per destination batch row ({B})")
    p = hip.IefAttnF32Params()
    res = hip._fill_attn(p, g, heads, scale, q, k, v, q_src, k_src, v_src, out=out,
                         out_planes=out_planes if dest is dest_p else False)
    if idx:
        hip._devi32(q_idx, "q_idx"), hip._devi32(k_idx, "k_idx")
        if q_idx.dim() != 1 or k_idx.dim() != 1 or not 1 <= q_idx.numel() <= N or not 1 <= k_idx.numel() <= L:
            raise ValueError("planes.attn_flash: q_idx / k_idx must be non-empty 1-D lists no longer than the operand's rows")
        p.N, p.L = N, L = q_idx.numel(), k_idx.numel()
        p.q_idx, p.k_idx = q_idx.data_ptr(), k_idx.data_ptr()
    if cls:
        hip._devi32(q_cls, "q_cls"), hip._devi32(k_cls, "k_cls")
        if N % 32 or L % 32 or q_cls.numel() != N // 32 or k_cls.numel() != L // 32:
            raise ValueError(f"planes.attn_flash: q_cls / k_cls hold one word per 32 tokens ({N} queries, {L} keys: multiples of 32)")
        p.q_cls, p.k_cls = q_cls.data_ptr(), k_cls.data_ptr()
    p.gate = _ptr(hip._devi32(gate, "gate"))
    if uni:
        hip._devi32(k2_src, "k2_src"), hip._devi32(v2_src, "v2_src")
        if k2_src.numel() != B or v2_src.numel() != B:
            raise ValueError(f"planes.attn_flash: k2_src / v2_src must have one entry per batch row ({B})")
        p.k2_src, p.v2_src = k2_src.data_ptr(), v2_src.data_ptr()
    p.zeros = _zeros(q.device)
    if lse is not None:
        p.lse = hip._dev32(lse, "lse").data_ptr()
    S = 1 if key_splits == 1 else attn_key_splits(B, heads, N, L, d, setting=key_splits)
    name, nbytes = f"attn_flash_x3p_kernel<{d}>", 4.0 * B * heads * d * (2 * N + 2 * L)
    if idx:
        name = f"attn_flash_x3p_kernel<{d}, idx>"
    elif cls:
        name = f"attn_flash_x3p_kernel<{d}, cls>"
    elif uni:
        name = f"attn_flash_x3p_kernel<{d}, uni>"
    elif S > 1:
        nws = lib.ief_attn_flash_ws_floats(B, heads, N, L, d, S)
        ws = torch.empty(nws, dtype=torch.float32, device=q.device)
        p.key_splits, p.ws, p.ws_floats = S, ws.data_ptr(), nws
        name, nbytes = f"attn_flash_x3p_kernel<{d}, split {S}> + attn_flash_x3p_combine_kernel", nbytes + 8.0 * nws
    with _Timed(name, 4.0 * B * heads * N * L * d, nbytes):
        _check(lib.ief_attn_flash_f32(byref(p), _stream()), "ief_attn_flash_f32 (planes)")
    return res
```

image-editing-framework_amd/unet.py:

```python
import math
import os
from typing import Dict, Optional

import torch
from torch import nn

from . import hip, planes
from .config import UNetConfig


FOLD_LN = os.environ.get("IEF_FOLD_LN", "1") == "1"
KV_ONE_GEMM = os.environ.get("IEF_KV_ONE_GEMM", "1") == "1"


def _fold_ln(w16, bias32, gamma, beta):
    wf = w16.float()
    wp = (wf * gamma[None, :]).half().contiguous()
    b = wf @ beta
    if bias32 is not None:
        b = b + bias32
    return wp, b.contiguous(), wp.float().sum(1).contiguous()


class UNetOutput(dict):

    def __getattr__(self, k):
        try:
            return self[k]
        except KeyError as e:
            raise AttributeError(k) from e


_PACK = torch.float16


def _f16(t, dev):
    return t.detach().to(device=dev, dtype=_PACK).contiguous()


def _f32(t, dev):
    return t.detach().to(device=dev, dtype=torch.float32).contiguous()


class Linear(nn.Module):
    def __init__(self, weight, bias=None):
        super().__init__()
        self.weight = weight
        self.bias = bias
        self.out_features, self.in_features = weight.shape

    def forward(self, x, residual=None):
        return hip.gemm(x, self.weight, bias=self.bias, residual=residual)


class Conv2d(nn.Module):

    def __init__(self, weight, bias, kernel_size, stride=1):
        super().__init__()
        self.weight, self.bias = weight, bias
        self.kernel_size, self.stride = kernel_size, stride

    def forward(self, x, **kw):
        if self.kernel_size == 1:
            return hip.gemm(x, self.weight, bias=self.bias, residual=kw.get("residual"), col_stats=kw.get("col_stats", False))
        return hip.conv3x3(x, self.weight, self.bias, stride=self.stride, **kw)


class GroupNorm(nn.Module):
    def __init__(self, weight, bias, num_groups, eps):
        super().__init__()
        self.weight, self.bias, self.num_groups, self.eps = weight, bias, num_groups, eps

    def forward(self, x, silu=False, x2=None, return_stats=False, cstat=None, cstat2=None):
        return hip.groupnorm(x, self.weight, self.bias, self.num_groups, self.eps, silu=silu, x2=x2, return_stats=return_stats,
                             cstat=cstat, cstat2=cstat2)


class LayerNorm(nn.Module):
    def __init__(self, weight, bias, eps=1e-5):
        super().__init__()
        self.weight, self.bias, self.eps = weight, bias, eps

    def forward(self, x):
        return hip.layernorm(x, self.weight, self.bias, self.eps)


class SiLU(nn.Module):
    def forward(self, x):
        return hip.silu(x)


class Dropout(nn.Module):
    def forward(self, x):
        return x


class Attention(nn.Module):

    def __init__(self, sd, prefix, dim, heads, cross_dim, dev, name):
        super().__init__()
        self.heads = heads
        self.inner_dim = dim
        self.dim_head = dim // heads
        self.scale = self.dim_head ** -0.5
        self.is_cross = cross_dim is not None
        self.layer_name = name
        wq, wk, wv = (_f16(sd[f"{prefix}.to_{n}.weight"], dev) for n in "qkv")
        if self.is_cross:
            self.w_kv = torch.cat([wk, wv], 0).contiguous()
            self.to_q = Linear(wq)
            self.to_k, self.to_v = Linear(self.w_kv[:dim]), Linear(self.w_kv[dim:])
            self.w_qkv = None
        else:
            self.w_qkv = torch.cat([wq, wk, wv], 0).contiguous()
            self.to_q, self.to_k, self.to_v = (Linear(self.w_qkv[i * dim:(i + 1) * dim]) for i in range(3))
            self.w_kv = None
        self.to_out = nn.ModuleList([
            Linear(_f16(sd[f"{prefix}.to_out.0.weight"], dev), _f32(sd[f"{prefix}.to_out.0.bias"], dev)), Dropout()])
        self.spatial_norm = None
        self.group_norm = None
        self.norm_cross = None
        self.residual_connection = False
        self.rescale_output_factor = 1.0
        self.processor = None
        self._plan = None
        self.map_out = None
        self._kv_key, self._kv = None, None
        self.cache_kv = True
        self._kv_view = None
        self.ln_w = self.ln_b = self.ln_c1 = None
        self.ln_eps = 1e-5
        self.attn_key_splits = 1

    def fold_layernorm(self, norm):
        w = self.w_qkv if self.w_qkv is not None else self.to_q.weight
        self.ln_w, self.ln_b, self.ln_c1 = _fold_ln(w, None, norm.weight, norm.bias)
        self.ln_eps = norm.eps

    def prepare_attention_mask(self, attention_mask, target_length, batch_size, out_dim=3):
        if attention_mask is not None:
            raise NotImplementedError("attention masks are not on the reference path (always None)")
        return None

    def head_to_batch_dim(self, t, out_dim=3):
        B, L, _ = t.shape
        t = t.reshape(B, L, self.heads, self.dim_head).permute(0, 2, 1, 3)
        return t.reshape(B * self.heads, L, self.dim_head) if out_dim == 3 else t

    def batch_to_head_dim(self, t):
        BH, L, d = t.shape
        B = BH // self.heads
        return t.reshape(B, self.heads, L, d).permute(0, 2, 1, 3).reshape(B, L, self.heads * d)

    def get_attention_scores(self, query, key, attention_mask=None):
        if attention_mask is not None:
            raise NotImplementedError("attention masks are not on the reference path")
        q = self.batch_to_head_dim(query).contiguous()
        k = self.batch_to_head_dim(key).contiguous()
        return hip.attn_probs(q, k, self.heads, self.scale)

    def apply_probs(self, probs, value):
        v = self.batch_to_head_dim(value).contiguous()
        return hip.attn_apply(probs.contiguous(), v, self.heads)

    def get_processor(self):
        return self.processor

    def set_processor(self, processor):
        self.processor = processor

    def is_native(self) -> bool:
        f = self.__dict__.get("forward")
        return (f is None or getattr(f, "__func__", None) is Attention.forward) and self.processor is None

    def context_kv(self, ctx):
        if self._kv_view is not None:
            return self._kv_view
        if not self.cache_kv:
            return hip.gemm(ctx, self.w_kv)
        key = (ctx, ctx._version)
        if self._kv_key is None or self._kv_key[0] is not ctx or self._kv_key[1] != ctx._version:
            self._kv = hip.gemm(ctx, self.w_kv)
            self._kv_key = key
        return self._kv

    def forward(self, hidden_states, encoder_hidden_states=None, attention_mask=None, temb=None, residual=None,
                ln_stats=None, want_stats=False, **cross_attention_kwargs):
        if self.processor is not None:
            return self.processor(self, hidden_states, encoder_hidden_states=encoder_hidden_states,
                                  attention_mask=attention_mask, **cross_attention_kwargs)
        x = hidden_states
        B, N, C = x.shape
        self.last_tokens = N
        plan = self._plan
        ln = None if ln_stats is None else (ln_stats, self.ln_c1, self.ln_eps)
        if encoder_hidden_states is None:
            qkv = hip.gemm(x, self.w_qkv) if ln is None else hip.gemm(x, self.ln_w, bias=self.ln_b, ln=ln)
            q, k, v = qkv[..., :C], qkv[..., C:2 * C], qkv[..., 2 * C:]
            qs = ks = vs = None
            if plan is not None:
                qs, ks, vs = plan.self_sources(B, N, self)
                if plan.second_sources(B, self) is not None:
                    raise RuntimeError(f"{self.layer_name}: the Union plan's two key segments exist on the planes attention of the "
                                       "f16x3 mode only")
            o = hip.attn_flash(q, k, v, self.heads, self.scale, q_src=qs, k_src=ks, v_src=vs)
        else:
            q = hip.gemm(x, self.to_q.weight) if ln is None else hip.gemm(x, self.ln_w, bias=self.ln_b, ln=ln)
            kv = self.context_kv(encoder_hidden_states)
            args = plan.cross_edit(B, self) if plan is not None else {}
            if self.map_out is not None:
                hip.attn_probs(q, kv[..., :C], self.heads, self.scale, out=self.map_out)
            o = hip.attn_cross_p2p(q, kv[..., :C], kv[..., C:], self.heads, self.scale, **args)
        if plan is not None:
            plan.layer_done(self)
        lin = self.to_out[0]
        if want_stats:
            return hip.gemm(o, lin.weight, bias=lin.bias, residual=residual, row_stats=True)
        return lin(o, residual=residual)


    def fold_layernorm_x3p(self, norm):
        w = self.w_qkv if self.w_qkv is not None else self.to_q.weight
        self.ln3 = planes.FoldedLN(w, None, norm.weight, norm.bias, norm.eps)

    def forward_x3p(self, xp, ctx, residual, ln_stats=None, want_stats=False, cfg_rows=None):
        B, N, C = xp.shape
        if cfg_rows is not None:
            if cfg_rows.rows != B:
                raise ValueError("forward_x3p: cfg_rows was built for another batch")
            B = cfg_rows.n
        self.last_tokens = N
        plan = self._plan
        w_in, b_in, ln = (self.w_qkv if ctx is None else self.to_q.weight), None, None
        if ln_stats is not None:
            w_in, b_in, ln = self.ln3.w, self.ln3.bias, (ln_stats, self.ln3.colsum, self.ln3.eps)
        if ctx is None:
            qs = ks = vs = None
            if plan is not None:
                qs, ks, vs = plan.self_sources(B, N, self)
            if cfg_rows is not None and (qs is not None or ks is not None or vs is not None
                                         or (plan is not None and plan.mask_launches(B, N, self) is not None)
                                         or (plan is not None and plan.kind == "masactrl_mask_auto"
                                             and (self._exec_index // 2) in plan.masa_layers)):
                raise RuntimeError(f"{self.layer_name}: the control plan acts on a self-attention that runs in the shared prefix of a "
                                   "CFG step (ControlPlan.controls_first_self must say so)")
            if planes.FLASH_PLANES and self.dim_head in planes.FLASH_PLANES_DIMS:
                qkv = planes.gemm(xp, w_in, bias=b_in, ln=ln, out=False, out_planes=True)
                k2 = plan.second_sources(B, self) if plan is not None else None
                if k2 is not None:
                    o = planes.attn_flash(qkv[..., :C], qkv[..., C:2 * C], qkv[..., 2 * C:], self.heads, self.scale, q_src=qs,
                                          k_src=ks, v_src=vs, k2_src=k2, v2_src=k2, key_splits=1)
                else:
                    o = planes.attn_flash(qkv[..., :C], qkv[..., C:2 * C], qkv[..., 2 * C:], self.heads, self.scale, q_src=qs,
                                          k_src=ks, v_src=vs, key_splits=self.attn_key_splits)
                ml = plan.mask_launches(B, N, self) if plan is not None else None
                if ml is not None:
                    tgt, src, gate, pairs = ml
                    for q_idx, k_idx in pairs:
                        planes.attn_flash(qkv[..., :C], qkv[..., C:2 * C], qkv[..., 2 * C:], self.heads, self.scale, q_src=tgt,
                                          k_src=src, v_src=src, out_planes=o[1::2], q_idx=q_idx, k_idx=k_idx, gate=gate)
                al = plan.auto_launch(B, N, self) if plan is not None else None
                if al is not None:
                    tgt, src, gate, k_cls, q_cls = al
                    planes.attn_flash(qkv[..., :C], qkv[..., C:2 * C], qkv[..., 2 * C:], self.heads, self.scale, q_src=tgt,
                                      k_src=src, v_src=src, out_planes=o[1::2], q_cls=q_cls, k_cls=k_cls, gate=gate)
            else:
                qkv = planes.gemm(xp, w_in, bias=b_in, ln=ln)
                if plan is not None and (plan.mask_launches(B, N, self) is not None or plan.auto_launch(B, N, self) is not None):
                    raise RuntimeError(f"mask-guided MasaCtrl was lowered onto a layer of head dim {self.dim_head} that has no "
                                       "planes attention")
                if plan is not None and plan.second_sources(B, self) is not None:
                    raise RuntimeError(f"MasaCtrl Union was lowered onto a layer of head dim {self.dim_head} that has no planes "
                                       "attention")
                o = hip.attn_flash(qkv[..., :C], qkv[..., C:2 * C], qkv[..., 2 * C:], self.heads, self.scale, q_src=qs, k_src=ks,
                                   v_src=vs, out_planes=True)
        else:
            q = planes.gemm(xp, w_in, bias=b_in, ln=ln)
            kv = self.context_kv(ctx)
            args = plan.cross_edit(B, self) if plan is not None else {}
            if self.map_out is not None:
                hip.attn_probs(q, kv[..., :C], self.heads, self.scale, out=self.map_out)
            if plan is not None:
                plan.cross_mass(B, N, self, q, kv[..., :C])
            o = hip.attn_cross_p2p(q, kv[..., :C], kv[..., C:], self.heads, self.scale, out_planes=True, q_src=cfg_rows, **args)
        if plan is not None:
            plan.layer_done(self)
        lin = self.to_out[0]
        if want_stats:
            return planes.gemm(o, lin.weight, bias=lin.bias, residual=residual, out=True, out_planes=True, row_stats=True)
        return planes.gemm(o, lin.weight, bias=lin.bias, residual=residual)


class GEGLU(nn.Module):

    def __init__(self, sd, prefix, dev):
        super().__init__()
        w, b = sd[prefix + ".proj.weight"], sd[prefix + ".proj.bias"]
        half = w.shape[0] // 2
        il = lambda t: torch.stack([t[:half].reshape(half // 8, 8, *t.shape[1:]),
                                    t[half:].reshape(half // 8, 8, *t.shape[1:])], 1).reshape(t.shape)
        self.proj = Linear(_f16(il(w), dev), _f32(il(b), dev))
        self.proj.interleaved = True

    def fold_layernorm(self, norm):
        self.ln_w, self.ln_b, self.ln_c1 = _fold_ln(self.proj.weight, self.proj.bias, norm.weight, norm.bias)
        self.ln_eps = norm.eps

    def forward(self, x, ln_stats=None):
        if ln_stats is not None:
            return hip.gemm(x, self.ln_w, bias=self.ln_b, geglu=True, ln=(ln_stats, self.ln_c1, self.ln_eps))
        return hip.gemm(x, self.proj.weight, bias=self.proj.bias, geglu=True)


class FeedForward(nn.Module):
    def __init__(self, sd, prefix, dev):
        super().__init__()
        self.net = nn.ModuleList([GEGLU(sd, prefix + ".net.0", dev), Dropout(),
                                  Linear(_f16(sd[prefix + ".net.2.weight"], dev), _f32(sd[prefix + ".net.2.bias"], dev))])

    def forward(self, x, residual=None):
        return self.net[2](self.net[0](x), residual=residual)


class BasicTransformerBlock(nn.Module):
    def __init__(self, sd, prefix, dim, heads, cross_dim, dev, name):
        super().__init__()
        ln = lambda n: LayerNorm(_f32(sd[f"{prefix}.{n}.weight"], dev), _f32(sd[f"{prefix}.{n}.bias"], dev))
        self.norm1, self.norm2, self.norm3 = ln("norm1"), ln("norm2"), ln("norm3")
        self.attn1 = Attention(sd, prefix + ".attn1", dim, heads, None, dev, name + ".attn1")
        self.attn2 = Attention(sd, prefix + ".attn2", dim, heads, cross_dim, dev, name + ".attn2")
        self.ff = FeedForward(sd, prefix + ".ff", dev)
        if dev.type == "cuda" and _PACK == torch.float16:
            self.attn1.fold_layernorm(self.norm1)
            self.attn2.fold_layernorm(self.norm2)
            self.ff.net[0].fold_layernorm(self.norm3)

    def foldable(self):
        return FOLD_LN and self.attn1.ln_w is not None and self.attn1.is_native() and self.attn2.is_native()

    @staticmethod
    def _attend(attn, x, res, ctx):
        if attn.is_native():
            return attn(x, encoder_hidden_states=ctx, residual=res)
        out = attn(x, encoder_hidden_states=ctx)
        return hip.add(out.contiguous(), res)

    def forward(self, h, ctx, ln_stats=None, want_stats=False):
        if ln_stats is not None:
            h, st = self.attn1(h, residual=h, ln_stats=ln_stats, want_stats=True)
            h, st = self.attn2(h, encoder_hidden_states=ctx, residual=h, ln_stats=st, want_stats=True)
            g = self.ff.net[0](h, ln_stats=st)
            lin = self.ff.net[2]
            if want_stats:
                return hip.gemm(g, lin.weight, bias=lin.bias, residual=h, row_stats=True)
            return lin(g, residual=h)
        h = self._attend(self.attn1, self.norm1(h), h, None)
        h = self._attend(self.attn2, self.norm2(h), h, ctx)
        return self.ff(self.norm3(h), residual=h)


    def _attend_x3p(self, attn, norm, h, ctx):
        if attn.is_native():
            return attn.forward_x3p(planes.layernorm(h, norm.weight, norm.bias, norm.eps), ctx, residual=h)
        return self._attend(attn, norm(h), h, ctx)

    def fold_layernorm_x3p(self):
        self.attn1.fold_layernorm_x3p(self.norm1)
        self.attn2.fold_layernorm_x3p(self.norm2)
        f0 = self.ff.net[0].proj
        self.ff.net[0].ln3 = planes.FoldedLN(f0.weight, f0.bias, self.norm3.weight, self.norm3.bias, self.norm3.eps)

    def foldable_x3p(self):
        if not (planes.LN_FOLD and self.attn1.is_native() and self.attn2.is_native()):
            return False
        if getattr(self.attn1, "ln3", None) is None:
            if hip._capturing():
                return False
            self.fold_layernorm_x3p()
        return True

    def forward_x3p_folded(self, h, hp, st, ctx, last, want_stats):
        h, hp, st = self.attn1.forward_x3p(hp, None, residual=h, ln_stats=st, want_stats=True)
        h, hp, st = self.attn2.forward_x3p(hp, ctx, residual=h, ln_stats=st, want_stats=True)
        f0, lin = self.ff.net[0], self.ff.net[2]
        g = planes.gemm(hp, f0.ln3.w, bias=f0.ln3.bias, geglu=True, out=False, out_planes=True, ln=(st, f0.ln3.colsum, f0.ln3.eps))
        if last:
            return planes.gemm(g, lin.weight, bias=lin.bias, residual=h, out=False, out_planes=True)
        if want_stats:
            return planes.gemm(g, lin.weight, bias=lin.bias, residual=h, out=True, out_planes=True, row_stats=True)
        return planes.gemm(g, lin.weight, bias=lin.bias, residual=h)

    def forward_x3p(self, h, ctx, last, cfg_rows=None, carry=()):
        if cfg_rows is not None:
            h = self.attn1.forward_x3p(planes.layernorm(h, self.norm1.weight, self.norm1.bias, self.norm1.eps), None, residual=h,
                                       cfg_rows=cfg_rows)
            n2 = planes.layernorm(h, self.norm2.weight, self.norm2.bias, self.norm2.eps)
            rep = hip.repeat_batch(h, *carry)
            h, carry = (rep[0], tuple(rep[1:])) if carry else (rep, ())
            h = self.attn2.forward_x3p(n2, ctx, residual=h, cfg_rows=cfg_rows)
        else:
            h = self._attend_x3p(self.attn1, self.norm1, h, None)
            h = self._attend_x3p(self.attn2, self.norm2, h, ctx)
        n3 = planes.layernorm(h, self.norm3.weight, self.norm3.bias, self.norm3.eps)
        f0, lin = self.ff.net[0].proj, self.ff.net[2]
        g = planes.gemm(n3, f0.weight, bias=f0.bias, geglu=True, out=False, out_planes=True)
        if last:
            r = planes.gemm(g, lin.weight, bias=lin.bias, residual=h, out=False, out_planes=True)
        else:
            r = planes.gemm(g, lin.weight, bias=lin.bias, residual=h)
        return (r, carry) if cfg_rows is not None else r


class Transformer2DModel(nn.Module):
    def __init__(self, sd, prefix, dim, heads, cross_dim, groups, dev, name, depth=1):
        super().__init__()
        self.norm = GroupNorm(_f32(sd[prefix + ".norm.weight"], dev), _f32(sd[prefix + ".norm.bias"], dev), groups, 1e-6)
        c1 = lambda n: Conv2d(_f16(sd[f"{prefix}.{n}.weight"].reshape(dim, dim), dev), _f32(sd[f"{prefix}.{n}.bias"], dev), 1)
        self.proj_in, self.proj_out = c1("proj_in"), c1("proj_out")
        self.transformer_blocks = nn.ModuleList(
            [BasicTransformerBlock(sd, f"{prefix}.transformer_blocks.{k}", dim, heads, cross_dim, dev,
                                   name if k == 0 else f"{name}.b{k}") for k in range(depth)])

    def forward(self, x, encoder_hidden_states=None, cstat=None, col_stats=False):
        B, H, W, C = x.shape
        if all(blk.foldable() for blk in self.transformer_blocks):
            h, st = hip.gemm(self.norm(x, cstat=cstat), self.proj_in.weight, bias=self.proj_in.bias, row_stats=True)
            h = h.reshape(B, H * W, C)
            last = len(self.transformer_blocks) - 1
            for k, blk in enumerate(self.transformer_blocks):
                if k < last:
                    h, st = blk(h, encoder_hidden_states, ln_stats=st, want_stats=True)
                else:
                    h = blk(h, encoder_hidden_states, ln_stats=st)
            return self.proj_out(h.reshape(B, H, W, C), residual=x, col_stats=col_stats)
        h = self.proj_in(self.norm(x, cstat=cstat)).reshape(B, H * W, C)
        for blk in self.transformer_blocks:
            h = blk(h, encoder_hidden_states)
        return self.proj_out(h.reshape(B, H, W, C), residual=x, col_stats=col_stats)


    def forward_x3p(self, x, encoder_hidden_states=None, want_planes=False, cfg_rows=None, carry=()):
        B, H, W, C = x.shape
        n = self.norm
        hn = planes.groupnorm(x, n.weight, n.bias, n.num_groups, n.eps, silu=False)
        last = len(self.transformer_blocks) - 1
        if cfg_rows is not None:
            h = planes.gemm(hn.reshape(B, H * W, C), self.proj_in.weight, bias=self.proj_in.bias)
            for k, blk in enumerate(self.transformer_blocks):
                if k == 0:
                    h, rep = blk.forward_x3p(h, encoder_hidden_states, last=(k == last), cfg_rows=cfg_rows, carry=(x,) + tuple(carry))
                    x, carry = rep[0], rep[1:]
                    B = x.shape[0]
                else:
                    h = blk.forward_x3p(h, encoder_hidden_states, last=(k == last))
        elif all(blk.foldable_x3p() for blk in self.transformer_blocks):
            h, hp, st = planes.gemm(hn.reshape(B, H * W, C), self.proj_in.weight, bias=self.proj_in.bias, out=True, out_planes=True,
                                    row_stats=True)
            for k, blk in enumerate(self.transformer_blocks):
                r = blk.forward_x3p_folded(h, hp, st, encoder_hidden_states, last=(k == last), want_stats=(k < last))
                if k < last:
                    h, hp, st = r
                else:
                    h = r
        else:
            h = planes.gemm(hn.reshape(B, H * W, C), self.proj_in.weight, bias=self.proj_in.bias)
            for k, blk in enumerate(self.transformer_blocks):
                h = blk.forward_x3p(h, encoder_hidden_states, last=(k == last))
        r = planes.gemm(h, self.proj_out.weight, bias=self.proj_out.bias, residual=x.reshape(B, H * W, C), out=True,
                        out_planes=want_planes)
        if want_planes:
            r = r[0].reshape(B, H, W, C), r[1].reshape(B, H, W, C)
        else:
            r = r.reshape(B, H, W, C), None
        return r + (tuple(carry),) if cfg_rows is not None else r


class ResnetBlock2D(nn.Module):

    def __init__(self, sd, prefix, cin, cout, groups, eps, dev, temb_slot):
        super().__init__()
        self.in_channels, self.out_channels = cin, cout
        self.norm1 = GroupNorm(_f32(sd[prefix + ".norm1.weight"], dev), _f32(sd[prefix + ".norm1.bias"], dev), groups, eps)
        self.norm2 = GroupNorm(_f32(sd[prefix + ".norm2.weight"], dev), _f32(sd[prefix + ".norm2.bias"], dev), groups, eps)
        pack = lambda w: _f16(w.permute(0, 2, 3, 1), dev)
        self.conv1 = Conv2d(pack(sd[prefix + ".conv1.weight"]), _f32(sd[prefix + ".conv1.bias"], dev), 3)
        self.time_emb_proj = Linear(_f16(sd[prefix + ".time_emb_proj.weight"], dev), _f32(sd[prefix + ".time_emb_proj.bias"], dev))
        self.nonlinearity = SiLU()
        self.dropout = Dropout()
        self.upsample = self.downsample = None
        self.skip_time_act = False
        self.time_embedding_norm = "default"
        self.output_scale_factor = 1.0
        w2 = sd[prefix + ".conv2.weight"].permute(0, 2, 3, 1).reshape(cout, 9 * cout)
        b2 = sd[prefix + ".conv2.bias"]
        if cin != cout:
            ws = sd[prefix + ".conv_shortcut.weight"].reshape(cout, cin)
            self.conv_shortcut = Conv2d(_f16(ws, dev), _f32(sd[prefix + ".conv_shortcut.bias"], dev), 1)
            self.w2_fused = _f16(torch.cat([w2, ws], 1), dev)
            self.b2_fused = _f32(b2 + sd[prefix + ".conv_shortcut.bias"], dev)
        else:
            self.conv_shortcut = None
            self.w2_fused, self.b2_fused = None, None
        self.conv2 = Conv2d(_f16(w2.reshape(cout, 3, 3, cout), dev), _f32(b2, dev), 3)
        self.temb_slot = temb_slot
        self._inject = None

    def forward(self, x, temb_row, skip=None, cstat=None, cstat_skip=None, col_stats=False):
        h = self.norm1(x, silu=True, x2=skip, cstat=cstat, cstat2=cstat_skip)
        h, hs = hip.conv3x3(h, self.conv1.weight, self.conv1.bias, rowvec=temb_row, col_stats=True)
        h = self.norm2(h, silu=True, cstat=hs)
        if self._inject is not None:
            src = self._inject.feature_source(h.shape[0])
            if src is not None:
                h = hip.gather_rows(h, src)
        if self.conv_shortcut is None:
            return hip.conv3x3(h, self.conv2.weight, self.conv2.bias, residual=x, col_stats=col_stats)
        return hip.conv3x3_shortcut(h, self.w2_fused, self.b2_fused, x, skip, col_stats=col_stats)


    def forward_x3p(self, x, xp, temb_row, skip=None, skip_p=None, want_planes=False):
        n1, n2 = self.norm1, self.norm2
        g1 = planes.groupnorm(x, n1.weight, n1.bias, n1.num_groups, n1.eps, silu=True, x2=skip)
        h = planes.conv3x3(g1, self.conv1.weight, self.conv1.bias, rowvec=temb_row)
        if self._inject is not None and self._inject.feature_source(h.shape[0]) is not None:
            g2 = planes.split(hip.gather_rows(hip.groupnorm(h, n2.weight, n2.bias, n2.num_groups, n2.eps, silu=True),
                                              self._inject.feature_source(h.shape[0])))
        else:
            g2 = planes.groupnorm(h, n2.weight, n2.bias, n2.num_groups, n2.eps, silu=True)
        if self.conv_shortcut is None:
            r = planes.conv3x3(g2, self.conv2.weight, self.conv2.bias, residual=x, out=True, out_planes=want_planes)
        else:
            xp = planes.split(x) if xp is None else xp
            if skip is not None and skip_p is None:
                skip_p = planes.split(skip)
            r = planes.conv3x3(g2, self.w2_fused, self.b2_fused, extra=(xp, skip_p), out=True, out_planes=want_planes)
        return r if want_planes else (r, None)


class Downsample2D(nn.Module):
    def __init__(self, sd, prefix, dev):
        super().__init__()
        self.conv = Conv2d(_f16(sd[prefix + ".conv.weight"].permute(0, 2, 3, 1), dev), _f32(sd[prefix + ".conv.bias"], dev), 3, stride=2)

    def forward(self, x, col_stats=False):
        return self.conv(x, col_stats=col_stats)

    def forward_x3p(self, xp, want_planes=True):
        r = planes.conv3x3(xp, self.conv.weight, self.conv.bias, stride=2, out=True, out_planes=want_planes)
        return r if want_planes else (r, None)


class Upsample2D(nn.Module):

    def __init__(self, sd, prefix, dev):
        super().__init__()
        self.conv = Conv2d(_f16(sd[prefix + ".conv.weight"].permute(0, 2, 3, 1), dev), _f32(sd[prefix + ".conv.bias"], dev), 3)

    def forward(self, x, col_stats=False):
        return hip.conv3x3(x, self.conv.weight, self.conv.bias, upsample=True, col_stats=col_stats)

    def forward_x3p(self, xp, want_planes=True):
        r = planes.conv3x3(xp, self.conv.weight, self.conv.bias, upsample=True, out=True, out_planes=want_planes)
        return r if want_planes else (r, None)


class _Block(nn.Module):
    def __init__(self):
        super().__init__()
        self.resnets = nn.ModuleList()
        self.attentions = nn.ModuleList()
        self.has_cross_attention = False


class CrossAttnDownBlock2D(_Block):
    pass


class DownBlock2D(_Block):
    pass


class CrossAttnUpBlock2D(_Block):
    pass


class UpBlock2D(_Block):
    pass


class UNetMidBlock2DCrossAttn(_Block):
    pass


class Timesteps(nn.Module):
    def __init__(self, dim):
        super().__init__()
        self.num_channels = dim
        self.dtype = _PACK

    def forward(self, t):
        return hip.timestep_embedding(t, self.num_channels, dtype=self.dtype)


class TimestepEmbedding(nn.Module):
    def __init__(self, sd, dev, prefix="time_embedding"):
        super().__init__()
        self.linear_1 = Linear(_f16(sd[prefix + ".linear_1.weight"], dev), _f32(sd[prefix + ".linear_1.bias"], dev))
        self.act = SiLU()
        self.linear_2 = Linear(_f16(sd[prefix + ".linear_2.weight"], dev), _f32(sd[prefix + ".linear_2.bias"], dev))

    def forward(self, x):
        return self.linear_2(self.act(self.linear_1(x)))


class UNet2DConditionModel(nn.Module):
    def __init__(self, cfg: UNetConfig, state_dict: Dict[str, torch.Tensor], device="cuda:0", precision: str = "f16",
                 attn_key_splits=1):
        super().__init__()
        global _PACK
        if precision not in ("f16", "f32", "f16x3"):
            raise ValueError('precision must be "f16", "f32" or "f16x3"')
        self.precision = precision
        self.contract = "x3" if precision == "f16x3" else "f32"
        saved, _PACK = _PACK, (torch.float16 if precision == "f16" else torch.float32)
        try:
            self._build(cfg, state_dict, device)
        finally:
            _PACK = saved
        self.attn_key_splits = attn_key_splits

    @property
    def attn_key_splits(self):
        return self._attn_key_splits

    @attn_key_splits.setter
    def attn_key_splits(self, v):
        self._attn_key_splits = planes.key_split_setting(v)
        for m in self.modules():
            if isinstance(m, Attention):
                m.attn_key_splits = self._attn_key_splits

    def _build(self, cfg, state_dict, device):
        hip.load()
        dev = torch.device(device)
        sd = state_dict
        self.cfg = cfg
        self.config = _Config(cfg)
        self._device = dev
        self.dtype = _PACK
        ch = cfg.block_out_channels
        nlev = len(ch)
        G, eps = cfg.norm_num_groups, cfg.norm_eps
        self.conv_in = Conv2d(_f16(sd["conv_in.weight"].permute(2, 3, 1, 0), dev), _f32(sd["conv_in.bias"], dev), 3)
        self.time_proj = Timesteps(ch[0])
        self.time_embedding = TimestepEmbedding(sd, dev)
        if cfg.addition_embed:
            self.add_time_proj = Timesteps(cfg.addition_time_embed_dim)
            self.add_embedding = TimestepEmbedding(sd, dev, "add_embedding")
        self._temb_width = 0
        self._resnets = []

        def resnet(prefix, cin, cout):
            r = ResnetBlock2D(sd, prefix, cin, cout, G, eps, dev, (self._temb_width, cout))
            self._temb_width += cout
            self._resnets.append(r)
            return r

        self.down_blocks = nn.ModuleList()
        cout = ch[0]
        for i in range(nlev):
            cin, cout = cout, ch[i]
            blk = CrossAttnDownBlock2D() if cfg.down_has_attn[i] else DownBlock2D()
            blk.has_cross_attention = cfg.down_has_attn[i]
            for j in range(cfg.layers_per_block):
                blk.resnets.append(resnet(f"down_blocks.{i}.resnets.{j}", cin if j == 0 else cout, cout))
                if cfg.down_has_attn[i]:
                    blk.attentions.append(Transformer2DModel(sd, f"down_blocks.{i}.attentions.{j}", cout, cfg.num_heads[i],
                                                             cfg.cross_attention_dim, G, dev, f"down{i}.{j}", cfg.depth(i)))
            blk.downsamplers = nn.ModuleList([Downsample2D(sd, f"down_blocks.{i}.downsamplers.0", dev)]) if i < nlev - 1 else None
            self.down_blocks.append(blk)
        self.up_blocks = nn.ModuleList()
        rev, rev_attn, rev_heads = tuple(reversed(ch)), tuple(reversed(cfg.down_has_attn)), tuple(reversed(cfg.num_heads))
        out_c = rev[0]
        up_specs = []
        for i in range(nlev):
            prev, out_c = out_c, rev[i]
            in_c = rev[min(i + 1, nlev - 1)]
            up_specs.append((i, prev, out_c, in_c))
        cm = ch[-1]
        self.mid_block = UNetMidBlock2DCrossAttn()
        self.mid_block.has_cross_attention = True
        self.mid_block.resnets.append(resnet("mid_block.resnets.0", cm, cm))
        self.mid_block.attentions.append(Transformer2DModel(sd, "mid_block.attentions.0", cm, cfg.num_heads[-1],
                                                            cfg.cross_attention_dim, G, dev, "mid", cfg.depth(nlev - 1)))
        self.mid_block.resnets.append(resnet("mid_block.resnets.1", cm, cm))
        for i, prev, out_c, in_c in up_specs:
            blk = CrossAttnUpBlock2D() if rev_attn[i] else UpBlock2D()
            blk.has_cross_attention = rev_attn[i]
            blk.skip_channels = []
            for j in range(cfg.layers_per_block + 1):
                skip = in_c if j == cfg.layers_per_block else out_c
                rin = prev if j == 0 else out_c
                blk.skip_channels.append(skip)
                blk.resnets.append(resnet(f"up_blocks.{i}.resnets.{j}", rin + skip, out_c))
                if rev_attn[i]:
                    blk.attentions.append(Transformer2DModel(sd, f"up_blocks.{i}.attentions.{j}", out_c, rev_heads[i],
                                                             cfg.cross_attention_dim, G, dev, f"up{i}.{j}",
                                                             cfg.depth(nlev - 1 - i)))
            blk.upsamplers = nn.ModuleList([Upsample2D(sd, f"up_blocks.{i}.upsamplers.0", dev)]) if i < nlev - 1 else None
            self.up_blocks.append(blk)
        self.conv_norm_out = GroupNorm(_f32(sd["conv_norm_out.weight"], dev), _f32(sd["conv_norm_out.bias"], dev), G, eps)
        self.conv_act = SiLU()
        self.conv_out = Conv2d(_f16(sd["conv_out.weight"].permute(0, 2, 3, 1), dev), _f32(sd["conv_out.bias"], dev), 3)
        self._temb_w = torch.cat([r.time_emb_proj.weight for r in self._resnets], 0).contiguous()
        self._temb_b = torch.cat([r.time_emb_proj.bias for r in self._resnets], 0).contiguous()
        order = [m for blk in self.down_blocks for m in blk.modules() if m.__class__.__name__ == "Attention"]
        order += [m for m in self.mid_block.modules() if m.__class__.__name__ == "Attention"]
        order += [m for blk in self.up_blocks for m in blk.modules() if m.__class__.__name__ == "Attention"]
        for i, m in enumerate(order):
            m._exec_index = i
        self.x3p = (self.precision == "f16x3" and planes.ENABLED and dev.type == "cuda"
                    and all(c % 160 == 0 or c % 64 == 0 for c in ch) and cfg.cross_attention_dim % 32 == 0)
        self._temb_table = None
        self._temb_static = None
        self._plan = None

    @property
    def device(self):
        return self._device

    def attention_modules(self):
        out = []
        for name, child in self.named_children():
            if "down" in name or "up" in name or "mid" in name:
                out += [m for m in child.modules() if m.__class__.__name__ == "Attention"]
        return out

    def packed_tensors(self):
        seen, out = set(), []
        holders = list(self.modules()) + [self]
        for m in holders:
            for v in vars(m).values():
                if isinstance(v, torch.Tensor) and v.is_cuda and v._base is None and v.data_ptr() not in seen:
                    seen.add(v.data_ptr())
                    out.append(v)
        return out

    def aug_embedding(self, added_cond_kwargs):
        with hip.f32_contraction(self.contract):
            return self._aug_embedding(added_cond_kwargs)

    def time_rows(self, timesteps_f32, aug=None):
        with hip.f32_contraction(self.contract):
            return self._time_rows(timesteps_f32, aug)

    def forward(self, sample, timestep=None, encoder_hidden_states=None, cross_attention_kwargs=None,
                added_cond_kwargs=None, return_dict=True, temb_row=None, taps=None, cfg_pair=False, **kw):
        with hip.f32_contraction(self.contract):
            return self._forward(sample, timestep, encoder_hidden_states, cross_attention_kwargs, added_cond_kwargs,
                                 return_dict, temb_row, taps, cfg_pair=cfg_pair, **kw)

    def cfg_shared_facts(self, latent_hw, ctx_len=77):
        blk = self.down_blocks[0]
        att = [m for m in blk.modules() if isinstance(m, Attention)]
        cross = bool(blk.has_cross_attention) and len(blk.attentions) > 0
        plan = self._plan
        return dict(x3p=bool(self.x3p), aug=bool(self.cfg.addition_embed), first_block_cross=cross,
                    native=all(m.is_native() for m in att),
                    fused_cross=cross and hip.cross_p2p_x3_ok(att[1].dim_head, ctx_len) and hip.FLASH_F32 and hip.X3_FUSE_CROSS,
                    ln_folded=bool(planes.LN_FOLD),
                    plan_on_first_self=plan is not None and plan.controls_first_self(self, int(latent_hw[0]) * int(latent_hw[1])))

    def _aug_embedding(self, added_cond_kwargs):
        if not self.cfg.addition_embed:
            return None
        if added_cond_kwargs is None:
            raise ValueError("this UNet has an additional text-time embedding: added_cond_kwargs is required")
        te = added_cond_kwargs["text_embeds"].to(self._device).float().contiguous()
        ids = added_cond_kwargs["time_ids"].to(self._device).float().contiguous()
        B = te.shape[0]
        tim = self.add_time_proj(ids.reshape(-1).contiguous()).reshape(B, -1)
        return self.add_embedding(torch.cat([self._act(te), tim], dim=-1).contiguous())

    def _time_rows(self, timesteps_f32, aug=None):
        emb = self.time_embedding(self.time_proj(timesteps_f32))
        if aug is not None:
            T, B = emb.shape[0], aug.shape[0]
            emb = hip.add(emb[:, None, :].expand(T, B, -1).contiguous(), aug[None].expand(T, B, -1).contiguous())
            emb = emb.reshape(T * B, -1)
        rows = hip.gemm(hip.silu(emb), self._temb_w, bias=self._temb_b)
        return rows if rows.dtype == torch.float32 else hip.to_f32(rows)

    def precompute_time_table(self, timesteps):
        t = torch.as_tensor(timesteps).to(device=self._device, dtype=torch.float32).reshape(-1).contiguous()
        self._temb_table = self.time_rows(t).contiguous()
        self._temb_static = torch.empty(1, self._temb_width, dtype=torch.float32, device=self._device)
        return self._temb_table

    def _forward(self, sample, timestep=None, encoder_hidden_states=None, cross_attention_kwargs=None,
                 added_cond_kwargs=None, return_dict=True, temb_row=None, taps=None, cfg_pair=False, **kw):
        if not sample.is_cuda:
            raise RuntimeError("UNet input must be a device tensor (no CPU path)")
        x = sample if sample.dtype == torch.float32 else sample.float()
        x = x.contiguous()
        ctx = encoder_hidden_states
        if cfg_pair:
            from .denoise import cfg_shared_prefix_reason
            if ctx.shape[0] != 2 * x.shape[0]:
                raise ValueError(f"cfg_pair: {x.shape[0]} latents stand for {2 * x.shape[0]} batch rows, the context has {ctx.shape[0]}")
            if cfg_shared_prefix_reason(mode="denoise", cfg=True, taps=taps is not None,
                                        **self.cfg_shared_facts(x.shape[-2:], ctx.shape[1])) is not None:
                x, cfg_pair = torch.cat([x, x]), False
        B = x.shape[0] * (2 if cfg_pair else 1)
        if ctx.dtype != self.dtype:
            ctx = self._ctx_f16(ctx)
        if temb_row is None:
            t = torch.as_tensor(timestep).to(device=self._device, dtype=torch.float32).reshape(-1)[:1].contiguous()
            temb_row = self.time_rows(t, self.aug_embedding(added_cond_kwargs))
        trow = lambda r: temb_row[:, r.temb_slot[0]:r.temb_slot[0] + r.temb_slot[1]].contiguous()
        if self._plan is not None:
            self._plan.begin_forward(B)
        cross = self._cross_modules()
        per_step_kv = KV_ONE_GEMM and bool(cross) and not cross[0].cache_kv and all(m.is_native() for m in cross)
        if per_step_kv:
            kv_all = hip.gemm(ctx, self._kv_all_weight())
            off = 0
# ... 129 lines not shown
```

include/ief_hip.h:

```cpp
#ifndef IEF_HIP_H
#define IEF_HIP_H
#include <stdint.h>

#ifdef __HIPCC__
typedef _Float16 ief_half;
#else
typedef uint16_t ief_half;
#endif

#ifdef __cplusplus
extern "C" {
#endif

#define IEF_ABI_VERSION 4
int ief_abi_version(void);
const char* ief_target_arch(void);
int ief_struct_size(int which);

typedef struct IefGemmParams {
    const ief_half* A;
    const ief_half* A2;
    const ief_half* W;
    ief_half* Out;
    const float* bias;
    const float* rowvec;
    const ief_half* residual;
    int M, N, K;
    int lda, ldw, ldo, ldr;
    long long strideA, strideW, strideO, strideR;
    int H, Wd, C1, C2, Ho, Wo, stride, ups, batch_images;
    int rows_per_batch;
    float out_scale;
    int tile_hint;
    const ief_half* E1; const ief_half* E2;
    int CE1, CE2;
    int splits;
    float* ws;
    int flags;
    const ief_half* zeros;
    int stages;
    int pad_hi_only;
    float* rstat_out;
    const float* rstat_in;
    int rstat_slots;
    const float* colsum;
    float ln_eps;
    float* cstat_out;
    int* cnt;
} IefGemmParams;

int ief_gemm_f16(const IefGemmParams* p, int batch, void* stream);
int ief_gemm_tile_bn(int tile_hint);
int ief_conv3x3_f16(const IefGemmParams* p, void* stream);

int ief_conv_in_f32(const float* x, const ief_half* w, const float* bias, ief_half* out,
                    int B, int Cin, int H, int Wd, int Cout, void* stream);
int ief_conv_out_f32(const ief_half* x, const ief_half* w, const float* bias, float* out,
                     int B, int C, int H, int Wd, int Cout, void* stream);

int ief_gn_splits(int HW);
int ief_groupnorm_silu_f16(const ief_half* x, const ief_half* x2, int C1, int C2, ief_half* out,
                           const float* gamma, const float* beta, float* partial,
                           int B, int HW, int groups, float eps, int apply_silu, void* stream);
int ief_layernorm_f16(const ief_half* x, ief_half* out, const float* gamma, const float* beta,
                      int rows, int C, float eps, void* stream);
int ief_geglu_f16(const ief_half* in, ief_half* out, int rows, int Ch, void* stream);

typedef struct IefAttnParams {
    const ief_half* Q; const ief_half* K; const ief_half* V; ief_half* Out;
    int B, heads, N, L, d;
    int ldq, ldk, ldv, ldo;
    float scale;
    const int* q_src; const int* k_src; const int* v_src;
    float* lse;
    int variant;
} IefAttnParams;
int ief_attn_flash_f16(const IefAttnParams* p, void* stream);

typedef struct IefCrossParams {
    const ief_half* Q; const ief_half* K; const ief_half* V; ief_half* Out;
    int B, heads, N, L, d;
    int ldq, ldk, ldv, ldo;
    float scale;
    const int* edit_src; const int* edit_slot;
    const ief_half* MT; const float* coef;
} IefCrossParams;
int ief_attn_cross_p2p_f16(const IefCrossParams* p, void* stream);

int ief_attn_probs_f16(const IefAttnParams* p, ief_half* probs, void* stream);
int ief_attn_apply_f16(const IefAttnParams* p, const ief_half* probs, void* stream);

int ief_cfg_ddim_step_f32(const float* eps_u, const float* eps_c, const float* x, float* x_out,
                          float* x0_out, const float* coef, long long n, void* stream);
int ief_cfg_ddim_step_rect_f32(const float* eps_u, const float* eps_c, const float* x, float* x_out, float* x0_out,
                               const float* coef, long long n, long long row_elems,
                               const float* traj, int traj_rows, const int* step, void* stream);
int ief_cfg_ddpm_step_f32(const float* eps_u, const float* eps_c, const float* x, float* x_out, float* x0_out, const float* coef,
                          const float* g_rows, long long n, long long row_elems,
                          const float* noise, int noise_rows, const int* step, void* stream);
int ief_ddpm_noise_maps_f32(const float* eps_u, const float* eps_c, const float* x_t, const float* x_prev, float* z_out,
                            const float* coef_rows, int R, long long row_elems, void* stream);
int ief_cfg_dpmpp_step_f32(const float* eps_u, const float* eps_c, const float* x, float* x_out, float* x0_out, float* x0_prev,
                           const float* coef, const float* g_rows, long long n, long long row_elems,
                           const float* noise, int noise_rows, const int* step, void* stream);
int ief_dpmpp_noise_maps_f32(const float* eps_u, const float* eps_c, const float* x_t, const float* x_prev, float* z_out,
                             const float* coef_rows, float* x0_carry, int R, long long row_elems, void* stream);
int ief_cfg_ddim_step_masked_f32(const float* eps_u, const float* eps_c, const float* x, float* x_out, float* x0_out,
                                 const float* coef, long long n, long long row_elems, long long hw,
                                 const float* traj, int traj_rows, const int* step, const float* mask, void* stream);
int ief_diffedit_map_accum_f32(const float* eps_a, const float* eps_b, float* acc, int R, int C, int hw, void* stream);
int ief_diffedit_mask_f32(const float* acc, float* mask_out, int hw, int count, float ratio, float thres, void* stream);
int ief_ledits_attn_mask_f32(const float* acc, const float* taps, const float* rank, float* m1_out, int E, void* stream);
int ief_ledits_guidance_mask_f32(const float* eps, const float* m1, const float* rank, float* mask_out, float* thres_out, int E,
                                 int C, int H, int W, void* stream);
int ief_ledits_ddpm_step_f32(const float* eps, const float* mask, const float* scale, const float* x, float* x_out, float* x0_out,
                             const float* coef, long long row_elems, long long hw, const float* noise, int noise_rows,
                             const int* step, int E, void* stream);
int ief_ledits_dpmpp_step_f32(const float* eps, const float* mask, const float* scale, const float* x, float* x_out, float* x0_out,
                              float* x0_prev, const float* coef, long long row_elems, long long hw, const float* noise,
                              int noise_rows, const int* step, int E, void* stream);
int ief_timestep_embedding_f16(const float* t, ief_half* out, int B, int dim, void* stream);
int ief_add_f16(const ief_half* a, const ief_half* b, ief_half* out, long long n, void* stream);
int ief_gather_rows_f16(const ief_half* in, ief_half* out, const int* src, int B, long long row_elems, void* stream);
int ief_softmax_rows_f16(ief_half* x, int rows, int L, void* stream);
int ief_transpose_f16(const ief_half* in, ief_half* out, int R, int C, void* stream);
int ief_pointwise_f32(const float* x, const float* w, const float* bias, float* out, int B, int Cin, int Cout, int HW,
                      void* stream);
int ief_silu_f16(const ief_half* x, ief_half* out, long long n, void* stream);
int ief_cast_f32_to_f16(const float* x, ief_half* out, long long n, void* stream);
int ief_cast_f16_to_f32(const ief_half* x, float* out, long long n, void* stream);
int ief_select_step(const void* table, void* out, const int* step, long long bytes_per_step, int n_rows, void* stream);
int ief_advance_step(int* step, void* stream);

typedef struct IefGemmF32Params {
    const float* A;
    const float* A2;
    const float* W;
    float* Out;
    const float* bias;
    const float* rowvec;
    const float* residual;
    int M, N, K;
    int lda, ldw, ldo, ldr;
    int rows_per_batch;
    float out_scale;
    int conv, H, Wd, C1, C2, Ho, Wo, stride, ups, batch_images, pad_hi_only;
    const float* E1;
    const float* E2;
    int CE1, CE2;
    int batch, heads;
    long long sAb, sAh, sWb, sWh, sOb, sOh;
    const int* a_src;
    const int* w_src;
    int transb;
    int a_scalar;
    int splits;
    float* ws;
    int x3;
    float sa, sb;
    int vec_out, al32, fast_ok;
    unsigned bytesA, bytesW, bytesA2, bytesE1, bytesE2;
    const void* Wp;
    int geglu;
} IefGemmF32Params;
int ief_gemm_f32(const IefGemmF32Params* p, void* stream);
int ief_x3_split_weights(const float* w, void* planes, long long n, float scale, void* stream);
int ief_gemm_x3_bn(int N);
int ief_gemm_x3_bm(int M, int N);
int ief_gemm_x3_bn_k(int conv, int N, int K);
void ief_gemm_x3_set_variant(int bits);
int ief_gemm_f32_bn(int N);
typedef struct IefAttnF32Params {
    const float* Q; const float* K; const float* V; float* Out;
    int B, heads, N, L, d;
    int ldq, ldk, ldv, ldo;
    long long sQb, sKb, sVb, sOb;
    float scale;
    const int* q_src; const int* k_src; const int* v_src;
    int x3;
    ief_half* OutP;
    long long planeO, sOPb;
    int ldp;
    float p_scale;
    const ief_half* Qp; const ief_half* Kp; const ief_half* Vp;
    long long planeQ, planeK, planeV;
    const void* zeros;
    float* lse;
    int key_splits; float* ws; long long ws_floats;
    const int* k2_src; const int* v2_src;
    const unsigned* k_cls; const unsigned* q_cls;
    const int* q_idx; const int* k_idx; const int* gate;
} IefAttnF32Params;
int ief_attn_flash_f32(const IefAttnF32Params* p, void* stream);
int ief_cross_token_mass_f32(const float* q, const float* k, const float* w, float* out, int row_ref, int row_cur, int heads,
                             int N, int L, int d, int ldq, int ldk, long long sQb, long long sKb, float scale, void* stream);
int ief_masa_auto_classes(const float* slots, int c, const float* thres, int res, unsigned* k_cls, unsigned* q_cls,
                          const int* gate, void* stream);
int ief_cross_blend_mass_f32(const float* q, const float* k, const float* w, float* acc, int row0, int Bp, int heads, int N, int L,
                             int ldw, int d, int ldq, int ldk, long long sQb, long long sKb, float scale, void* stream);
int ief_local_blend_f32(const float* acc, const float* thres, float* x, int Bp, int C, int H, int W, void* stream);
long long ief_attn_flash_ws_floats(int B, int heads, int N, int L, int d, int key_splits);
int ief_softmax_rows_f32(float* x, long long rows, int L, void* stream);
int ief_p2p_cross_edit_f32(float* P, const int* edit_src, const int* edit_slot, const float* MT, const float* coef, int B,
                           int heads, int N, int L, void* stream);
int ief_attn_cross_p2p_f32(const IefAttnF32Params* p, const int* edit_src, const int* edit_slot, const float* MT, const float* coef,
                           void* stream);
int ief_groupnorm_silu_f32(const float* x, const float* x2, int C1, int C2, float* out, const float* gamma, const float* beta,
                           int B, int HW, int groups, float eps, int silu, void* stream);
long long ief_groupnorm_f32_ws_floats(int B, int HW, int C);
int ief_groupnorm_silu_f32_ws(const float* x, const float* x2, int C1, int C2, float* out, const float* gamma, const float* beta,
                              int B, int HW, int groups, float eps, int silu, float* ws, long long ws_floats, void* stream);
int ief_groupnorm_reg_fits(int C1, int C2, int HW, int groups);
int ief_groupnorm_silu_reg(const float* x, const float* x2, int C1, int C2, float* out, ief_half* outp, long long plane,
                           const float* gamma, const float* beta, int B, int HW, int groups, float eps, int silu, void* stream);
long long ief_groupnorm_bwd_f32_ws_floats(int B, int HW, int C);
int ief_groupnorm_bwd_f32_ws(const float* x, const float* x2, int C1, int C2, const float* dy, const float* add, float* dx, float* dx2,
                             const float* gamma, const float* beta, int B, int HW, int groups, float eps, int silu, float* ws,
                             long long ws_floats, void* stream);
int ief_layernorm_f32(const float* x, float* out, const float* gamma, const float* beta, long long rows, int C, float eps,
                      void* stream);
int ief_groupnorm_silu_x3p_ws(const float* x, const float* x2, int C1, int C2, float* out, ief_half* outp, long long plane,
                              const float* gamma, const float* beta, int B, int HW, int groups, float eps, int silu, float* ws,
                              long long ws_floats, void* stream);
int ief_groupnorm_silu_x3p_small(const float* x, const float* x2, int C1, int C2, ief_half* outp, long long plane, const float* gamma,
                                 const float* beta, int B, int HW, int groups, float eps, int silu, void* stream);
int ief_layernorm_x3p(const float* x, ief_half* outp, long long plane, const float* gamma, const float* beta, long long rows, int C,
                      float eps, void* stream);
int ief_add_f32(const float* a, const float* b, float* out, long long n, void* stream);
int ief_silu_f32(const float* x, float* out, long long n, void* stream);
int ief_geglu_il_f32(const float* pre, float* out, long long rows, int Ch, void* stream);
int ief_timestep_embedding_f32(const float* t, float* out, int B, int dim, void* stream);
int ief_gather_rows_f32(const float* in, float* out, const int* src, int B, long long row_elems, void* stream);
int ief_conv_in_f32act(const float* x, const float* w, const float* bias, float* out, int B, int Cin, int H, int Wd, int Cout,
                       void* stream);
int ief_conv_out_f32act(const float* x, const float* w, const float* bias, float* out, int B, int C, int H, int Wd, int Cout,
                        void* stream);
int ief_conv_in_f32act_planes(const float* x, const float* w, const float* bias, float* out, ief_half* outp, long long plane, int B,
                              int Cin, int H, int Wd, int Cout, void* stream);
#define IEF_REPEAT_MAX_JOBS 4
typedef struct IefRepeatJob { const void* src; void* dst; long long bytes; int blocks; } IefRepeatJob;
int ief_repeat_batch(const IefRepeatJob* jobs, int njobs, void* stream);
int ief_image_u8(const float* x, unsigned char* out, int B, int C, int H, int Wd, void* stream);

typedef struct IefGemmX3pParams {
    const ief_half* A;  long long planeA;
    const ief_half* A2; long long planeA2;
    const ief_half* E1; long long planeE1;
    const ief_half* E2; long long planeE2;
    const ief_half* W;  long long planeW;
    float* Out;
    ief_half* OutP; long long planeO;
    const float* bias;
    const float* rowvec;
    const float* residual;
    int M, N, K;
    int lda, ldw, ldo, ldp, ldr;
    int conv, H, Wd, C1, C2, Ho, Wo, stride, ups, batch_images, pad_hi_only, CE1, CE2;
    int rows_per_batch;
    float out_scale;
    float inv_scale;
    int tile;
    int splits;
    float* ws;
    int geglu;
    const void* zeros;
    float* rstat_out;
    float* cstat_out;
    const float* rstat_in;
    const float* colsum;
    int rstat_slots, rstat_cnt;
    float ln_eps;
} IefGemmX3pParams;
int ief_gemm_x3p(const IefGemmX3pParams* p, void* stream);
int ief_x3_upsample_phase_weights(const float* w, void* planes, int Cout, int C, float scale, void* stream);
int ief_gemm_x3p_tile_bm(int tile);
int ief_gemm_x3p_tile_bn(int tile);
int ief_gemm_x3p_tile_wn(int tile);
int ief_x3_split_act(const float* x, ief_half* planes, long long plane, long long rows, int C, int ldx, int ldp, float scale,
                     void* stream);

int ief_groupnorm_bwd_f32(const float* x, const float* x2, int C1, int C2, const float* dy, const float* add, float* dx, float* dx2,
                          const float* gamma, const float* beta, int B, int HW, int groups, float eps, int silu, void* stream);
int ief_layernorm_bwd_f32(const float* x, const float* dy, const float* add, float* dx, const float* gamma, long long rows, int C,
                          float eps, void* stream);
int ief_geglu_il_bwd_f32(const float* pre, const float* dy, float* dpre, long long rows, int Ch, void* stream);
int ief_zero_insert2x_f32(const float* in, float* out, int B, int H, int W, int C, void* stream);
int ief_pool2x2_sum_f32(const float* in, float* out, int B, int H, int W, int C, void* stream);
int ief_conv_out_bwd_f32w(const float* d_eps, const float* w, float* dh, int B, int C, int H, int W, int Cout, void* stream);
int ief_softmax_bwd_rows_f32(const float* P, float* dP, long long rows, int L, float scale, void* stream);
int ief_transpose_batched_f32(const float* in, float* out, int R, int N, int L, void* stream);
int ief_map_loss_rows_blocks(long long rows);
int ief_map_loss_rows_f32(const float* P, const float* ref, float* dP, float* loss, long long rows, int L, float gcoef,
                          float loss_coef, void* stream);
int ief_nti_adam_f32g(float* param, float* m, float* v, const float* grad, const float* stats, const float* hyper, int* step, int n,
                      void* stream);

typedef struct IefAttnBwdParams {
    const ief_half* Q; const ief_half* K; const ief_half* V; const ief_half* dO;
    const float* lse;
    const float* delta;
    ief_half* dQ; ief_half* dK; ief_half* dV;
    int B, heads, N, L, d;
    int ldq, ldk, ldv, ldo, lddq, lddk, lddv;
    float scale;
    float ds_mul;
    int kv_splits;
    float* ws;
} IefAttnBwdParams;
int ief_attn_bwd_delta_f32(const ief_half* O, const ief_half* dO, float* delta, int B, int heads, int N, int d,
                           int ldo, int lddo, void* stream);
int ief_attn_bwd_f16(const IefAttnBwdParams* p, int what, void* stream);
typedef struct IefAttnBwdF32Params {
    const float* Q; const float* K; const float* V; const float* dO;
    const float* lse;
    const float* delta;
    float* dQ; float* dK; float* dV;
    int B, heads, N, L, d;
    int ldq, ldk, ldv, ldo, lddq, lddk, lddv;
    float scale;
    float ds_mul;
} IefAttnBwdF32Params;
int ief_attn_bwd_delta_f32in(const float* O, const float* dO, float* delta, int B, int heads, int N, int d, int ldo, int lddo,
                             void* stream);
int ief_attn_bwd_x3(const IefAttnBwdF32Params* p, int what, void* stream);
typedef struct IefMapLossParams {
    const ief_half* Q; const ief_half* K; const ief_half* ref;
    ief_half* dQ;
    float* loss;
    int B, heads, N, L, d;
    int ldq, ldk, lddq;
    float scale, gcoef, loss_coef;
    int accumulate;
} IefMapLossParams;
int ief_attn_map_loss_bwd_f16(const IefMapLossParams* p, void* stream);
int ief_map_loss_blocks(int N, int d);
#define IEF_CROSS_MAP_GRAD_MAX_L 106
int ief_attn_cross_map_grad_f32(const float* Q, const float* K, const float* V, const float* dO, const float* ref, float* dQ,
                                float* loss, int B, int heads, int N, int L, int d, int ldq, int ldk, int ldv, int ldo, int lddq,
                                float scale, float gcoef, float loss_coef, void* stream);
int ief_cross_map_grad_blocks(int N, int d);
#define IEF_CROSS_BWD_MAX_L 80
int ief_attn_cross_bwd_f32(const float* Q, const float* K, const float* V, const float* dO, float* dQ, float* dK, float* dV,
                           float* scratch, int B, int heads, int N, int L, int d, int ldq, int ldk, int ldv, int ldo, int lddq,
                           int lddk, int lddv, float scale, void* stream);
int ief_cross_bwd_blocks(int N, int d);
long long ief_cross_bwd_scratch_floats(int B, int heads, int N, int L, int d);
int ief_axpy_f32(float* y, const float* x, float a, long long n, void* stream);
int ief_groupnorm_cstat_f16(const ief_half* x, const ief_half* x2, int C1, int C2, ief_half* out, const float* gamma,
                            const float* beta, const float* cstat1, int bm1, const float* cstat2, int bm2, float* stats,
                            int B, int HW, int groups, float eps, int apply_silu, void* stream);
int ief_gemm_tile_bm(int tile_hint);
int ief_groupnorm_bwd_f16(const ief_half* x, const ief_half* x2, int C1, int C2, const ief_half* dy, const ief_half* add,
                          ief_half* dx, ief_half* dx2, const float* gamma, const float* beta, const float* stats,
                          float* partial, int B, int HW, int groups, float eps, int apply_silu, void* stream);
int ief_layernorm_bwd_f16(const ief_half* x, const ief_half* dy, const ief_half* add, ief_half* dx, const float* gamma,
                          int rows, int C, float eps, void* stream);
int ief_geglu_il_f16(const ief_half* pre, ief_half* out, int rows, int Ch, void* stream);
int ief_geglu_il_bwd_f16(const ief_half* pre, const ief_half* dy, ief_half* dpre, int rows, int Ch, void* stream);
int ief_zero_insert2x_f16(const ief_half* in, ief_half* out, int B, int H, int W, int C, void* stream);
int ief_pool2x2_sum_f16(const ief_half* in, ief_half* out, int B, int H, int W, int C, void* stream);
int ief_conv_out_bwd_f32(const float* d_eps, const ief_half* w, ief_half* dh, int B, int C, int H, int W, int Cout,
                         void* stream);
int ief_nti_loss_grad_f32(const float* eps_u, const float* eps_c, const float* x, const float* target, const float* coef,
                          float* d_eps, float* stats, int n, float grad_scale, void* stream);
int ief_nti_adam_f32(float* param, float* m, float* v, const ief_half* grad16, const float* stats, const float* hyper,
                     int* step, ief_half* param16, int n, void* stream);
int ief_nti_loss_grad_batched_f32(const float* eps_u, const float* eps_c, const float* x, const float* target, const float* coef,
                                  float* d_eps, float* stats, int n, int K, float grad_scale, void* stream);
int ief_nti_adam_batched_f32(float* param, float* m, float* v, const ief_half* grad16, const float* stats, const int* active,
                             const float* hyper, int* step, ief_half* param16, int n, int K, void* stream);
int ief_nti_adam_batched_f32g(float* param, float* m, float* v, const float* grad, const float* stats, const int* active,
                              const float* hyper, int* step, int n, int K, void* stream);

#ifdef __cplusplus
}
#endif
#endif
```

Before: 81.25 steps/s.

## Fuse split-K slab reduction into following groupnorm/layernorm kernels

Split-K GEMMs can now stop after writing their partial slabs and return a deferred Slabs object. The next groupnorm or layernorm kernel sums the slabs, adds bias, rowvec and residual, optionally writes the fp32 sum, and emits the hi/lo fp16 planes. This removes a separate reduce kernel launch and one full fp32 write and re-read per fused GEMM-norm pair. The cost is more reads inside the norm kernels and higher register pressure, and it only applies when splits stay within a small limit.

Result: no change. 81.60 steps/s, median of 6 (+0.4%).

```diff
diff --git a/image-editing-framework_amd/csrc/exact_f32.hip b/image-editing-framework_amd/csrc/exact_f32.hip
--- a/image-editing-framework_amd/csrc/exact_f32.hip
+++ b/image-editing-framework_amd/csrc/exact_f32.hip
@@ -1201,6 +1201,164 @@
     return IEF_OK;
 }
 
+template <int E>
+__global__ __launch_bounds__(1024) void groupnorm_reg_slabs_kernel(const float* __restrict__ ws, int splits, long long slab,
+                                                                   const float* __restrict__ bias, const float* __restrict__ rowvec,
+                                                                   int rv_images, const float* __restrict__ residual, int ldr,
+                                                                   const float* __restrict__ x2, int C1, int C2,
+                                                                   float* __restrict__ sum_out, half_t* __restrict__ outp, long long plane,
+                                                                   const float* __restrict__ gamma, const float* __restrict__ beta, int HW,
+                                                                   int groups, float eps, int silu) {
+    typedef __attribute__((ext_vector_type(2))) float f32x2;
+    __shared__ float red[16];
+    __shared__ float bc;
+    __shared__ float sc_s[512], sh_s[512];
+    const int C = C1 + C2, cpg = C / groups, cp2 = cpg >> 1;
+    const int b = blockIdx.x / groups, g = blockIdx.x - b * groups;
+    const int npairs = HW * cp2;
+    const int tid = threadIdx.x;
+    const int dq = 1024 / cp2, dr = 1024 - dq * cp2;
+    int p = tid / cp2, j = tid - p * cp2;
+    f32x2 v[E];
+    const int p00 = p, j00 = j;
+    const float* wb = ws + (long long)b * HW * C1;
+    const float* x2b = x2 ? x2 + (long long)b * HW * C2 : wb;
+#pragma unroll
+    for (int k = 0; k < E; ++k) {
+        const bool ok = tid + k * 1024 < npairs;
+        const int c = g * cpg + (ok ? 2 * j : 0), pp = ok ? p : 0;
+        const float* src = c < C1 ? wb + (unsigned)(pp * C1 + c) : x2b + (unsigned)(pp * C2 + (c - C1));
+        const f32x2 t = *(const f32x2*)src;
+        v[k] = ok ? t : (f32x2){0.f, 0.f};
+        p += dq; j += dr;
+        if (j >= cp2) { j -= cp2; ++p; }
+        if ((k & 3) == 3) __builtin_amdgcn_sched_barrier(0);
+    }
+    if (tid < cpg && g * cpg + tid < C1) {
+        if (bias) sc_s[tid] = bias[g * cpg + tid];
+        if (rowvec) sh_s[tid] = rowvec[(long long)(b / rv_images) * C1 + g * cpg + tid];
+    }
+    auto add_pass = [&](const float* base, int ld, auto nsl) {
+        constexpr int S = decltype(nsl)::value;
+        f32x2 t[S][E];
+        bool s1[E];
+        p = p00; j = j00;
+        asm volatile("" : "+v"(p), "+v"(j));
+#pragma unroll
+        for (int k = 0; k < E; ++k) {
+            const int c = g * cpg + 2 * j;
+            s1[k] = tid + k * 1024 < npairs && c < C1;
+            const float* src = base + (s1[k] ? (unsigned)(p * ld + c) : 0u);
+#pragma unroll
+            for (int u = 0; u < S; ++u) t[u][k] = *(const f32x2*)(src + u * slab);
+            p += dq; j += dr;
+            if (j >= cp2) { j -= cp2; ++p; }
+            if ((k & 3) == 3) __builtin_amdgcn_sched_barrier(0);
+        }
+#pragma unroll
+        for (int u = 0; u < S; ++u) {
+#pragma unroll
+            for (int k = 0; k < E; ++k) {
+                const f32x2 a = v[k] + t[u][k];
+                v[k] = s1[k] ? a : v[k];
+            }
+        }
+    };
+    constexpr int SU = E == 4 ? 4 : E == 8 ? 3 : 1;
+    int si = 1;
+#pragma unroll 1
+    for (; si + SU - 1 < splits; si += SU) add_pass(wb + si * slab, C1, std::integral_constant<int, SU>{});
+#pragma unroll 1
+    for (; si < splits; ++si) add_pass(wb + si * slab, C1, std::integral_constant<int, 1>{});
+    if (bias || rowvec) {
+        __syncthreads();
+        j = j00;
+#pragma unroll
+        for (int k = 0; k < E; ++k) {
+            if (tid + k * 1024 < npairs && g * cpg + 2 * j < C1) {
+                if (bias) v[k] = v[k] + (f32x2){sc_s[2 * j], sc_s[2 * j + 1]};
+                if (rowvec) v[k] = v[k] + (f32x2){sh_s[2 * j], sh_s[2 * j + 1]};
+            }
+            j += dr;
+            if (j >= cp2) j -= cp2;
+        }
+    }
+    if (residual) add_pass(residual + (long long)b * HW * ldr, ldr, std::integral_constant<int, 1>{});
+    auto block_sum = [&](float t) -> float {
+        t = wave_sum(t);
+        __syncthreads();
+        if ((tid & 63) == 0) red[tid >> 6] = t;
+        __syncthreads();
+        if (tid == 0) { float a = 0.f; for (int w = 0; w < 16; ++w) a += red[w]; bc = a; }
+        __syncthreads();
+        return bc;
+    };
+    float s = 0.f;
+#pragma unroll
+    for (int k = 0; k < E; ++k) s += v[k][0] + v[k][1];
+    const float n = (float)cpg * (float)HW;
+    const float mean = block_sum(s) / n;
+    float q = 0.f;
+#pragma unroll
+    for (int k = 0; k < E; ++k) {
+        if (tid + k * 1024 < npairs) { const float d0 = v[k][0] - mean, d1 = v[k][1] - mean; q += d0 * d0 + d1 * d1; }
+    }
+    const float rstd = 1.0f / sqrtf(block_sum(q) / n + eps);
+    if (tid < cpg) {
+        const float sc = rstd * gamma[g * cpg + tid];
+        sc_s[tid] = sc;
+        sh_s[tid] = beta[g * cpg + tid] - mean * sc;
+    }
+    __syncthreads();
+    p = p00; j = j00;
+    asm volatile("" : "+v"(p), "+v"(j));
+    float* sb = sum_out ? sum_out + (long long)b * HW * C1 : nullptr;
+    half_t* opb = outp + (long long)b * HW * C;
+#pragma unroll
+    for (int k = 0; k < E; ++k) {
+        const int idx = tid + k * 1024;
+        if (idx < npairs) {
+            const int c = g * cpg + 2 * j;
+            if (sum_out && c < C1) *(f32x2*)(sb + (unsigned)(p * C1 + c)) = v[k];
+            float y0 = v[k][0] * sc_s[2 * j] + sh_s[2 * j], y1 = v[k][1] * sc_s[2 * j + 1] + sh_s[2 * j + 1];
+            if (silu) { y0 = silu_x(y0); y1 = silu_x(y1); }
+            const unsigned o = (unsigned)(p * C + c);
+            const half2_t h = __builtin_convertvector((f32x2){y0, y1}, half2_t);
+            const half2_t l = __builtin_convertvector((f32x2){y0 - (float)h[0], y1 - (float)h[1]}, half2_t);
+            *(half2_t*)(opb + o) = h;
+            *(half2_t*)(opb + plane + o) = l;
+        }
+        p += dq; j += dr;
+        if (j >= cp2) { j -= cp2; ++p; }
+        if ((k & 3) == 3) __builtin_amdgcn_sched_barrier(0);
+    }
+}
+extern "C" int ief_groupnorm_silu_reg_slabs(const float* ws, int splits, const float* bias, const float* rowvec, int rows_per_batch,
+                                            const float* residual, int ldr, const float* x2, int C1, int C2, float* sum_out,
+                                            ief_half* outp, long long plane, const float* gamma, const float* beta, int B, int HW,
+                                            int groups, float eps, int silu, void* stream) {
+    if (!ws || !outp || !gamma || !beta || (C2 > 0 && !x2) || splits < 2 || splits > 64) return IEF_EINVAL;
+    if (B <= 0 || HW <= 0 || !ief_groupnorm_reg_fits(C1, C2, HW, groups) || (plane & 1)) return IEF_ESHAPE;
+    if (rowvec && (rows_per_batch <= 0 || rows_per_batch % HW)) return IEF_ESHAPE;
+    if (residual && (ldr < C1 || (ldr & 1) || (long long)HW * ldr >= (1ll << 32))) return IEF_ESHAPE;
+    if ((((uintptr_t)ws | (uintptr_t)(x2 ? x2 : ws) | (uintptr_t)(sum_out ? sum_out : ws) | (uintptr_t)(bias ? bias : ws) |
+          (uintptr_t)(rowvec ? rowvec : ws) | (uintptr_t)(residual ? residual : ws)) & 7) || ((uintptr_t)outp & 3)) return IEF_EALIGN;
+    const int cpg = (C1 + C2) / groups;
+    const int need = (HW * (cpg >> 1) + 1023) / 1024;
+    const dim3 grid(B * groups), blk(1024);
+    hipStream_t st = (hipStream_t)stream;
+    const long long slab = (long long)B * HW * C1;
+    const int rv_images = rowvec ? rows_per_batch / HW : 1;
+#define GNS_GO(E_) hipLaunchKernelGGL(groupnorm_reg_slabs_kernel<E_>, grid, blk, 0, st, ws, splits, slab, bias, rowvec, rv_images, residual, ldr, x2, C1, C2, sum_out, (half_t*)outp, plane, gamma, beta, HW, groups, eps, silu)
+    if (need <= 4) GNS_GO(4);
+    else if (need <= 8) GNS_GO(8);
+    else if (need <= 16) GNS_GO(16);
+    else GNS_GO(20);
+#undef GNS_GO
+    IEF_LAUNCH_CHECK();
+    return IEF_OK;
+}
+
 __global__ __launch_bounds__(256) void layernorm_f32_kernel(const float* __restrict__ x, float* __restrict__ out,
                                                             const float* __restrict__ gamma, const float* __restrict__ beta,
                                                             long long rows, int C, float eps) {
@@ -1272,6 +1430,112 @@
     if (C <= 512) hipLaunchKernelGGL(layernorm_f32_vec_kernel<2>, grid, dim3(256), 0, st, x, none, gamma, beta, rows, C, eps, (half_t*)outp, plane);
     else if (C <= 1280) hipLaunchKernelGGL(layernorm_f32_vec_kernel<5>, grid, dim3(256), 0, st, x, none, gamma, beta, rows, C, eps, (half_t*)outp, plane);
     else hipLaunchKernelGGL(layernorm_f32_vec_kernel<10>, grid, dim3(256), 0, st, x, none, gamma, beta, rows, C, eps, (half_t*)outp, plane);
+    IEF_LAUNCH_CHECK();
+    return IEF_OK;
+}
+template <int NV>
+__global__ __launch_bounds__(256) void layernorm_slabs_vec_kernel(const float* __restrict__ ws, int splits, long long slab,
+                                                                  const float* __restrict__ bias, const float* __restrict__ residual,
+                                                                  int ldr, float* __restrict__ sum_out, const float* __restrict__ gamma,
+                                                                  const float* __restrict__ beta, long long rows, int C, float eps,
+                                                                  half_t* __restrict__ outp, long long plane) {
+    const long long row = (long long)blockIdx.x * 4 + (threadIdx.x >> 6);
+    if (row >= rows) return;
+    const float* r = ws + row * C;
+    const int lane = threadIdx.x & 63, CQ = C >> 2;
+    const f32x4 zero = {0.f, 0.f, 0.f, 0.f};
+    f32x4 v[NV], bb[NV], rb[NV];
+    const float* rr = residual + row * ldr;
+#pragma unroll
+    for (int j = 0; j < NV; ++j) {
+        const int qd = lane + 64 * j;
+        v[j] = qd < CQ ? *(const f32x4*)(r + qd * 4) : zero;
+        bb[j] = bias && qd < CQ ? *(const f32x4*)(bias + qd * 4) : zero;
+        rb[j] = residual && qd < CQ ? *(const f32x4*)(rr + qd * 4) : zero;
+    }
+    constexpr int SU = NV <= 5 ? 3 : 1;
+    int si = 1;
+#pragma unroll 1
+    for (; si + SU - 1 < splits; si += SU) {
+        f32x4 t[SU][NV];
+#pragma unroll
+        for (int u = 0; u < SU; ++u) {
+#pragma unroll
+            for (int j = 0; j < NV; ++j) {
+                const int qd = lane + 64 * j;
+                t[u][j] = qd < CQ ? *(const f32x4*)(r + (si + u) * slab + qd * 4) : zero;
+            }
+        }
+#pragma unroll
+        for (int u = 0; u < SU; ++u) {
+#pragma unroll
+            for (int j = 0; j < NV; ++j) v[j] += t[u][j];
+        }
+    }
+#pragma unroll 1
+    for (; si < splits; ++si) {
+        f32x4 t[NV];
+#pragma unroll
+        for (int j = 0; j < NV; ++j) {
+            const int qd = lane + 64 * j;
+            t[j] = qd < CQ ? *(const f32x4*)(r + si * slab + qd * 4) : zero;
+        }
+#pragma unroll
+        for (int j = 0; j < NV; ++j) v[j] += t[j];
+    }
+    if (bias) {
+#pragma unroll
+        for (int j = 0; j < NV; ++j) v[j] += bb[j];
+    }
+    if (residual) {
+#pragma unroll
+        for (int j = 0; j < NV; ++j) v[j] += rb[j];
+    }
+    float s = 0.f;
+#pragma unroll
+    for (int j = 0; j < NV; ++j) {
+        const int qd = lane + 64 * j;
+        if (sum_out && qd < CQ) *(f32x4*)(sum_out + row * C + qd * 4) = v[j];
+        s += (v[j][0] + v[j][1]) + (v[j][2] + v[j][3]);
+    }
+    const float mean = wave_sum(s) / (float)C;
+    float q = 0.f;
+#pragma unroll
+    for (int j = 0; j < NV; ++j) {
+        if (lane + 64 * j < CQ) {
+            const f32x4 d = v[j] - mean;
+            q += (d[0] * d[0] + d[1] * d[1]) + (d[2] * d[2] + d[3] * d[3]);
+        }
+    }
+    const float rstd = 1.0f / sqrtf(wave_sum(q) / (float)C + eps);
+#pragma unroll
+    for (int j = 0; j < NV; ++j) {
+        const int qd = lane + 64 * j;
+        if (qd < CQ) {
+            const f32x4 y = (v[j] - mean) * rstd * *(const f32x4*)(gamma + qd * 4) + *(const f32x4*)(beta + qd * 4);
+            half4 h, l;
+            split4(y, 1.0f, h, l);
+            half_t* op = outp + row * C + qd * 4;
+            *(half4*)op = h;
+            *(half4*)(op + plane) = l;
+        }
+    }
+}
+extern "C" int ief_layernorm_x3p_slabs(const float* ws, int splits, const float* bias, const float* residual, int ldr, float* sum_out,
+                                       ief_half* outp, long long plane, const float* gamma, const float* beta, long long rows, int C,
+                                       float eps, void* stream) {
+    if (!ws || !outp || !gamma || !beta || splits < 2 || splits > 64) return IEF_EINVAL;
+    if (rows <= 0 || C <= 0 || (C & 3) || C > 2560 || (plane & 3) || (residual && (ldr < C || (ldr & 3)))) return IEF_ESHAPE;
+    if ((((uintptr_t)ws | (uintptr_t)gamma | (uintptr_t)beta | (uintptr_t)(bias ? bias : ws) | (uintptr_t)(residual ? residual : ws) |
+          (uintptr_t)(sum_out ? sum_out : ws)) & 15) || ((uintptr_t)outp & 7)) return IEF_EALIGN;
+    const dim3 grid((unsigned)((rows + 3) / 4));
+    hipStream_t st = (hipStream_t)stream;
+    const long long slab = rows * C;
+#define LNS_GO(NV_) hipLaunchKernelGGL(layernorm_slabs_vec_kernel<NV_>, grid, dim3(256), 0, st, ws, splits, slab, bias, residual, ldr, sum_out, gamma, beta, rows, C, eps, (half_t*)outp, plane)
+    if (C <= 512) LNS_GO(2);
+    else if (C <= 1280) LNS_GO(5);
+    else LNS_GO(10);
+#undef LNS_GO
     IEF_LAUNCH_CHECK();
     return IEF_OK;
 }
diff --git a/image-editing-framework_amd/csrc/gemm_x3p.hip b/image-editing-framework_amd/csrc/gemm_x3p.hip
--- a/image-editing-framework_amd/csrc/gemm_x3p.hip
+++ b/image-editing-framework_amd/csrc/gemm_x3p.hip
@@ -465,11 +465,24 @@
     return IEF_OK;
 }
 
+static int x3p_reduce(const IefGemmX3pParams& p, hipStream_t st) {
+    const long long total = (long long)p.M * (p.N / 4);
+    int grid = (int)((total + 255) / 256);
+    if (grid > 8192) grid = 8192;
+    hipLaunchKernelGGL(x3p_reduce_kernel, dim3(grid), dim3(256), 0, st, p);
+    IEF_LAUNCH_CHECK();
+    return IEF_OK;
+}
+
 int ief_conv_halo_x3p_dispatch(const IefGemmX3pParams& p, hipStream_t st);
 
-extern "C" int ief_gemm_x3p(const IefGemmX3pParams* pp, void* stream) {
-    if (!pp || !pp->A || !pp->W || !pp->zeros || (!pp->Out && !pp->OutP)) return IEF_EINVAL;
+static int x3p_run(const IefGemmX3pParams* pp, void* stream, bool slabs_only) {
+    if (!pp || !pp->A || !pp->W || !pp->zeros || (!slabs_only && !pp->Out && !pp->OutP)) return IEF_EINVAL;
     IefGemmX3pParams p = *pp;
+    if (slabs_only) {
+        if (p.splits <= 1 || !p.ws) return IEF_EINVAL;
+        p.Out = nullptr; p.OutP = nullptr;
+    }
     if (p.M <= 0 || p.N <= 0 || p.K <= 0 || (p.K % XP_BK) || (p.N & 3)) return IEF_ESHAPE;
     if (p.rowvec && p.rows_per_batch <= 0) return IEF_ESHAPE;
     if (p.splits > 1 && (!p.ws || p.splits > 64 || p.geglu || p.rstat_out || p.cstat_out)) return IEF_EINVAL;
@@ -514,12 +527,19 @@
         case 1: default: rc = launch_x3p<128, 160, 4, 2, 4, 0>(p, st); break;
     }
     if (rc) return rc;
-    if (p.splits > 1) {
-        const long long total = (long long)p.M * (p.N / 4);
-        int grid = (int)((total + 255) / 256);
-        if (grid > 8192) grid = 8192;
-        hipLaunchKernelGGL(x3p_reduce_kernel, dim3(grid), dim3(256), 0, st, p);
-        IEF_LAUNCH_CHECK();
-    }
+    if (p.splits > 1 && !slabs_only) return x3p_reduce(p, st);
     return IEF_OK;
 }
+extern "C" int ief_gemm_x3p(const IefGemmX3pParams* pp, void* stream) { return x3p_run(pp, stream, false); }
+extern "C" int ief_gemm_x3p_slabs(const IefGemmX3pParams* pp, void* stream) { return x3p_run(pp, stream, true); }
+extern "C" int ief_gemm_x3p_reduce(const IefGemmX3pParams* pp, void* stream) {
+    if (!pp || !pp->ws || (!pp->Out && !pp->OutP)) return IEF_EINVAL;
+    const IefGemmX3pParams& p = *pp;
+    if (p.M <= 0 || p.N <= 0 || (p.N & 3) || (p.rowvec && p.rows_per_batch <= 0)) return IEF_ESHAPE;
+    if (p.splits <= 1 || p.splits > 64) return IEF_EINVAL;
+    if (p.Out && ((p.ldo & 3) || ((uintptr_t)p.Out & 15))) return IEF_EALIGN;
+    if (p.OutP && ((p.ldp & 3) || (p.planeO & 3) || ((uintptr_t)p.OutP & 7))) return IEF_EALIGN;
+    if (((uintptr_t)p.ws & 15) || (p.bias && ((uintptr_t)p.bias & 15)) || (p.rowvec && ((uintptr_t)p.rowvec & 15)) ||
+        (p.residual && (((uintptr_t)p.residual & 15) || (p.ldr & 3)))) return IEF_EALIGN;
+    return x3p_reduce(p, (hipStream_t)stream);
+}
diff --git a/image-editing-framework_amd/planes.py b/image-editing-framework_amd/planes.py
--- a/image-editing-framework_amd/planes.py
+++ b/image-editing-framework_amd/planes.py
@@ -258,8 +258,48 @@
 LN_FOLD = os.environ.get("IEF_X3P_FOLD_LN", "0") == "1"
 
 
+SLAB_NORM = os.environ.get("IEF_X3P_SLAB_NORM", "1") == "1"
+SLAB_NORM_MAX_SPLITS = int(os.environ.get("IEF_X3P_SLAB_NORM_MAX_SPLITS", "4"))
+
+
+class Slabs:
+    __slots__ = ("ws", "splits", "M", "N", "bias", "rowvec", "rows_per_batch", "residual", "shape")
+
+    def __init__(self, ws, splits, M, N, bias, rowvec, rows_per_batch, residual, shape):
+        self.ws, self.splits, self.M, self.N = ws, splits, M, N
+        self.bias, self.rowvec, self.rows_per_batch, self.residual = bias, rowvec, rows_per_batch, residual
+        self.shape = torch.Size(shape)
+
+    @property
+    def device(self):
+        return self.ws.device
+
+    def ldr(self):
+        return 0 if self.residual is None else hip._rows_ld32(self.residual, "residual")[2]
+
+    def reduce(self):
+        lib = hip.load()
+        out = torch.empty(self.shape, dtype=torch.float32, device=self.device)
+        p = IefGemmX3pParams()
+        p.M, p.N, p.splits, p.ws, p.out_scale = self.M, self.N, self.splits, self.ws.data_ptr(), 1.0
+        p.Out, p.ldo = out.data_ptr(), self.N
+        p.bias = _ptr(self.bias)
+        if self.rowvec is not None:
+            p.rowvec, p.rows_per_batch = self.rowvec.data_ptr(), self.rows_per_batch
+        if self.residual is not None:
+            p.residual, p.ldr = self.residual.data_ptr(), self.ldr()
+        with _Timed("x3p_reduce_kernel", 0.0, 4.0 * self.M * self.N * (self.splits + 1 + (1 if self.residual is not None else 0))):
+            _check(lib.ief_gemm_x3p_reduce(byref(p), _stream()), "ief_gemm_x3p_reduce")
+        return out
+
+
+def defers(splits, out=None, out_planes=None, out_scale=1.0, geglu=False, row_stats=False, ln=None):
+    return bool(SLAB_NORM and 1 < splits <= SLAB_NORM_MAX_SPLITS and out is None and out_planes in (None, False) and out_scale == 1.0
+                and not geglu and not row_stats and ln is None)
+
+
 def gemm(a, w, bias=None, residual=None, rowvec=None, rows_per_batch=0, out=None, out_planes=None, out_scale=1.0,
-         geglu=False, tile=0, splits=0, row_stats=False, ln=None):
+         geglu=False, tile=0, splits=0, row_stats=False, ln=None, defer=False):
     lib = hip.load()
     if not isinstance(a, Planes):
         raise TypeError("planes.gemm: a must be Planes")
@@ -272,7 +312,8 @@
     p.A, p.planeA, p.lda = a.t.data_ptr(), a.plane, lda
     p.W, p.planeW, p.ldw = wp.data_ptr(), wp.stride(0), K
     No = N // 2 if geglu else N
-    o32, op = _out_args(p, M, No, out, out_planes, a.device, a.shape[:-1])
+    may_defer = defer and defers(2, out, out_planes, out_scale, geglu, row_stats, ln)
+    o32, op = (None, None) if may_defer else _out_args(p, M, No, out, out_planes, a.device, a.shape[:-1])
     p.M, p.N, p.K = M, N, K
     p.out_scale, p.inv_scale = out_scale, 1.0 / (ACT_SCALE * W_SCALE)
     p.geglu, p.zeros = 1 if geglu else 0, _zeros(a.device)
@@ -299,11 +340,18 @@
         if st.buf.shape[0] != M or st.slots * st.cnt != K or _dev32(colsum, "colsum").numel() != N:
             raise ValueError("planes.gemm: ln statistics / colsum do not match this launch")
         p.rstat_in, p.rstat_slots, p.rstat_cnt, p.colsum, p.ln_eps = st.buf.data_ptr(), st.slots, st.cnt, colsum.data_ptr(), eps
+    slabs = may_defer and defers(p.splits)
+    if may_defer and not slabs:
+        o32, op = _out_args(p, M, No, out, out_planes, a.device, a.shape[:-1])
     ws = hip._fill_epilogue(p, hip._rows_ld32, "planes.gemm", M, N, a.device, bias, rowvec, rows_per_batch, residual, p.splits)
     nbytes = 4.0 * (M * K + N * K + M * No * ((1 if o32 is not None else 0) + (1 if op is not None else 0)) + (M * N if residual is not None else 0))
     kn = f"igemm_x3p_kernel<false> t{p.tile}" + (f" {M}x{N}x{K} s{p.splits}" if hip.PROF_SHAPES else "")
     bm, bn = _TILES[p.tile]
     hip.note_staged(kn, 4.0 * K * (bm + bn) * -(-M // bm) * -(-N // bn))
+    if slabs:
+        with _Timed(kn + (" slabs" if hip.PROF_SHAPES else ""), 2.0 * M * N * K, 4.0 * (M * K + N * K + p.splits * M * N)):
+            _check(lib.ief_gemm_x3p_slabs(byref(p), _stream()), "ief_gemm_x3p_slabs")
+        return Slabs(ws, p.splits, M, N, bias, rowvec, rows_per_batch, residual, tuple(a.shape[:-1]) + (N,))
     with _Timed(kn, 2.0 * M * N * K, nbytes):
         _check(lib.ief_gemm_x3p(byref(p), _stream()), "ief_gemm_x3p")
     r = _ret(o32, op)
@@ -313,7 +361,7 @@
 
 
 def conv3x3(x, w, bias=None, x2=None, stride=1, upsample=False, rowvec=None, residual=None, out=None, out_planes=None,
-            extra=None, pad_hi_only=False, tile=0, splits=0):
+            extra=None, pad_hi_only=False, tile=0, splits=0, defer=False):
     lib = hip.load()
     if not isinstance(x, Planes) or (x2 is not None and not isinstance(x2, Planes)):
         raise TypeError("planes.conv3x3: x / x2 must be Planes")
@@ -336,7 +384,8 @@
         p.E1, p.planeE1 = e1.t.data_ptr(), e1.plane
     if e2 is not None:
         p.E2, p.planeE2 = e2.t.data_ptr(), e2.plane
-    o32, op = _out_args(p, M, Cout, out, out_planes, x.device, (B, Ho, Wo))
+    may_defer = defer and defers(2, out, out_planes)
+    o32, op = (None, None) if may_defer else _out_args(p, M, Cout, out, out_planes, x.device, (B, Ho, Wo))
     p.M, p.N, p.K = M, Cout, K
     p.conv, p.H, p.Wd, p.C1, p.C2, p.Ho, p.Wo = 1, H, Wd, C1, C2, Ho, Wo
     p.stride, p.ups, p.batch_images, p.pad_hi_only = stride, 1 if upsample else 0, B, 1 if pad_hi_only else 0
@@ -379,6 +428,9 @@
             p.splits = min(p.splits, (C1 + C2) // 32)
         wp = weight_planes(w)
     p.W, p.planeW, p.ldw = wp.data_ptr(), wp.stride(0), K
+    slabs = may_defer and defers(p.splits)
+    if may_defer and not slabs:
+        o32, op = _out_args(p, M, Cout, out, out_planes, x.device, (B, Ho, Wo))
     ws = hip._fill_epilogue(p, hip._rows_ld32, "planes.conv3x3", M, Cout, x.device, bias, rowvec, g.rows_per_batch, residual, p.splits)
     nbytes = 4.0 * (B * Hp * Wp * (C1 + C2) + M * (CE1 + CE2) + Cout * K + M * Cout * ((1 if o32 is not None else 0) + (1 if op is not None else 0) + (1 if residual is not None else 0)))
     kn = "conv3x3_halo_x3p_kernel_phase" if p.tile == 13 else \
@@ -391,6 +443,11 @@
     else:
         bm, bn = _TILES[p.tile]
         hip.note_staged(kn, 4.0 * K * (bm + bn) * -(-M // bm) * -(-Cout // bn))
+    if slabs:
+        with _Timed(kn + (" slabs" if hip.PROF_SHAPES else ""), 2.0 * M * Cout * K,
+                    4.0 * (B * Hp * Wp * (C1 + C2) + M * (CE1 + CE2) + Cout * K + p.splits * M * Cout)):
+            _check(lib.ief_gemm_x3p_slabs(byref(p), _stream()), "ief_gemm_x3p_slabs (conv)")
+        return Slabs(ws, p.splits, M, Cout, bias, rowvec, g.rows_per_batch, residual, (B, Ho, Wo, Cout))
     with _Timed(kn, 2.0 * M * Cout * K, nbytes):
         _check(lib.ief_gemm_x3p(byref(p), _stream()), "ief_gemm_x3p (conv)")
     return _ret(o32, op)
@@ -402,8 +459,37 @@
 ENABLED = os.environ.get("IEF_X3P", "1") == "1"
 
 
-def groupnorm(x, gamma, beta, groups, eps, silu=False, x2=None, out32=False):
+def _groupnorm_slabs(h, gamma, beta, groups, eps, silu, x2, want_sum):
     lib = hip.load()
+    B, C1 = h.shape[0], h.N
+    C2 = 0 if x2 is None else x2.shape[-1]
+    HW = h.M // B
+    if not (HW <= GN_REG_MAX_HW and lib.ief_groupnorm_reg_fits(C1, C2, HW, groups)) or h.splits > SLAB_NORM_MAX_SPLITS:
+        return None
+    if h.rowvec is not None and (h.rows_per_batch <= 0 or h.rows_per_batch % HW):
+        return None
+    out = Planes.empty(*h.shape[:-1], C1 + C2, device=h.device)
+    s32 = torch.empty(h.shape, dtype=torch.float32, device=h.device) if want_sum else None
+    nbytes = 4.0 * (h.splits * h.M * C1 + (h.M * C1 if h.residual is not None else 0) + (h.M * C1 if want_sum else 0) + 2 * h.M * C2 + h.M * C1)
+    with _Timed("groupnorm_reg_slabs_kernel", 0.0, nbytes):
+        _check(lib.ief_groupnorm_silu_reg_slabs(h.ws.data_ptr(), h.splits, _ptr(h.bias), _ptr(h.rowvec), h.rows_per_batch,
+                                                _ptr(h.residual), h.ldr(), _ptr(x2), C1, C2, _ptr(s32), out.t.data_ptr(), out.plane,
+                                                _dev32(gamma, "gamma").data_ptr(), _dev32(beta, "beta").data_ptr(), B, HW, groups,
+                                                eps, 1 if silu else 0, _stream()), "ief_groupnorm_silu_reg_slabs")
+    return (out, s32) if want_sum else out
+
+
+def groupnorm(x, gamma, beta, groups, eps, silu=False, x2=None, out32=False, want_sum=False):
+    lib = hip.load()
+    if x2 is not None and not hip._act32(x2, "x2").is_contiguous():
+        raise ValueError("planes.groupnorm: inputs must be contiguous")
+    if isinstance(x, Slabs):
+        r = None if out32 else _groupnorm_slabs(x, gamma, beta, groups, eps, silu, x2, want_sum)
+        if r is not None:
+            return r
+        x = x.reduce()
+    if want_sum:
+        return groupnorm(x, gamma, beta, groups, eps, silu=silu, x2=x2, out32=out32), x
     if not hip._act32(x, "x").is_contiguous() or (x2 is not None and not hip._act32(x2, "x2").is_contiguous()):
         raise ValueError("planes.groupnorm: inputs must be contiguous")
     B, C1 = x.shape[0], x.shape[-1]
@@ -434,8 +520,22 @@
     return (out, o32) if out32 else out
 
 
-def layernorm(x, gamma, beta, eps=1e-5):
+def layernorm(x, gamma, beta, eps=1e-5, want_sum=False):
     lib = hip.load()
+    if isinstance(x, Slabs):
+        h, C = x, x.N
+        if h.rowvec is None and C % 4 == 0 and C <= 2560 and h.splits <= SLAB_NORM_MAX_SPLITS:
+            out = Planes.empty(*h.shape, device=h.device)
+            s32 = torch.empty(h.shape, dtype=torch.float32, device=h.device) if want_sum else None
+            nbytes = 4.0 * h.M * C * (h.splits + 1 + (1 if h.residual is not None else 0) + (1 if want_sum else 0))
+            with _Timed("layernorm_slabs_vec_kernel", 0.0, nbytes):
+                _check(lib.ief_layernorm_x3p_slabs(h.ws.data_ptr(), h.splits, _ptr(h.bias), _ptr(h.residual), h.ldr(), _ptr(s32),
+                                                   out.t.data_ptr(), out.plane, _dev32(gamma, "gamma").data_ptr(),
+                                                   _dev32(beta, "beta").data_ptr(), h.M, C, eps, _stream()), "ief_layernorm_x3p_slabs")
+            return (out, s32) if want_sum else out
+        x = h.reduce()
+    if want_sum:
+        return layernorm(x, gamma, beta, eps), x
     if not hip._act32(x, "x").is_contiguous():
         raise ValueError("planes.layernorm: x must be contiguous")
     C = x.shape[-1]
diff --git a/image-editing-framework_amd/unet.py b/image-editing-framework_amd/unet.py
--- a/image-editing-framework_amd/unet.py
+++ b/image-editing-framework_amd/unet.py
@@ -223,7 +223,7 @@
         w = self.w_qkv if self.w_qkv is not None else self.to_q.weight
         self.ln3 = planes.FoldedLN(w, None, norm.weight, norm.bias, norm.eps)
 
-    def forward_x3p(self, xp, ctx, residual, ln_stats=None, want_stats=False, cfg_rows=None):
+    def forward_x3p(self, xp, ctx, residual, ln_stats=None, want_stats=False, cfg_rows=None, defer=False):
         B, N, C = xp.shape
         if cfg_rows is not None:
             if cfg_rows.rows != B:
@@ -288,7 +288,7 @@
         lin = self.to_out[0]
         if want_stats:
             return planes.gemm(o, lin.weight, bias=lin.bias, residual=residual, out=True, out_planes=True, row_stats=True)
-        return planes.gemm(o, lin.weight, bias=lin.bias, residual=residual)
+        return planes.gemm(o, lin.weight, bias=lin.bias, residual=residual, defer=defer)
 
 
 class GEGLU(nn.Module):
@@ -359,9 +359,10 @@
         return self.ff(self.norm3(h), residual=h)
 
 
-    def _attend_x3p(self, attn, norm, h, ctx):
+    def _attend_x3p(self, attn, norm, h, ctx, defer=False):
         if attn.is_native():
-            return attn.forward_x3p(planes.layernorm(h, norm.weight, norm.bias, norm.eps), ctx, residual=h)
+            n, h = planes.layernorm(h, norm.weight, norm.bias, norm.eps, want_sum=True)
+            return attn.forward_x3p(n, ctx, residual=h, defer=defer)
         return self._attend(attn, norm(h), h, ctx)
 
     def fold_layernorm_x3p(self):
@@ -399,9 +400,9 @@
             h, carry = (rep[0], tuple(rep[1:])) if carry else (rep, ())
             h = self.attn2.forward_x3p(n2, ctx, residual=h, cfg_rows=cfg_rows)
         else:
-            h = self._attend_x3p(self.attn1, self.norm1, h, None)
-            h = self._attend_x3p(self.attn2, self.norm2, h, ctx)
-        n3 = planes.layernorm(h, self.norm3.weight, self.norm3.bias, self.norm3.eps)
+            h = self._attend_x3p(self.attn1, self.norm1, h, None, defer=self.attn2.is_native())
+            h = self._attend_x3p(self.attn2, self.norm2, h, ctx, defer=True)
+        n3, h = planes.layernorm(h, self.norm3.weight, self.norm3.bias, self.norm3.eps, want_sum=True)
         f0, lin = self.ff.net[0].proj, self.ff.net[2]
         g = planes.gemm(n3, f0.weight, bias=f0.bias, geglu=True, out=False, out_planes=True)
         if last:
@@ -463,7 +464,8 @@
                 else:
                     h = r
         else:
-            h = planes.gemm(hn.reshape(B, H * W, C), self.proj_in.weight, bias=self.proj_in.bias)
+            h = planes.gemm(hn.reshape(B, H * W, C), self.proj_in.weight, bias=self.proj_in.bias,
+                            defer=self.transformer_blocks[0].attn1.is_native())
             for k, blk in enumerate(self.transformer_blocks):
                 h = blk.forward_x3p(h, encoder_hidden_states, last=(k == last))
         r = planes.gemm(h, self.proj_out.weight, bias=self.proj_out.bias, residual=x.reshape(B, H * W, C), out=True,
@@ -521,7 +523,7 @@
     def forward_x3p(self, x, xp, temb_row, skip=None, skip_p=None, want_planes=False):
         n1, n2 = self.norm1, self.norm2
         g1 = planes.groupnorm(x, n1.weight, n1.bias, n1.num_groups, n1.eps, silu=True, x2=skip)
-        h = planes.conv3x3(g1, self.conv1.weight, self.conv1.bias, rowvec=temb_row)
+        h = planes.conv3x3(g1, self.conv1.weight, self.conv1.bias, rowvec=temb_row, defer=self._inject is None)
         if self._inject is not None and self._inject.feature_source(h.shape[0]) is not None:
             g2 = planes.split(hip.gather_rows(hip.groupnorm(h, n2.weight, n2.bias, n2.num_groups, n2.eps, silu=True),
                                               self._inject.feature_source(h.shape[0])))
diff --git a/include/ief_hip.h b/include/ief_hip.h
--- a/include/ief_hip.h
+++ b/include/ief_hip.h
@@ -272,6 +272,15 @@
     float ln_eps;
 } IefGemmX3pParams;
 int ief_gemm_x3p(const IefGemmX3pParams* p, void* stream);
+int ief_gemm_x3p_slabs(const IefGemmX3pParams* p, void* stream);
+int ief_gemm_x3p_reduce(const IefGemmX3pParams* p, void* stream);
+int ief_groupnorm_silu_reg_slabs(const float* ws, int splits, const float* bias, const float* rowvec, int rows_per_batch,
+                                 const float* residual, int ldr, const float* x2, int C1, int C2, float* sum_out, ief_half* outp,
+                                 long long plane, const float* gamma, const float* beta, int B, int HW, int groups, float eps, int silu,
+                                 void* stream);
+int ief_layernorm_x3p_slabs(const float* ws, int splits, const float* bias, const float* residual, int ldr, float* sum_out,
+                            ief_half* outp, long long plane, const float* gamma, const float* beta, long long rows, int C, float eps,
+                            void* stream);
 int ief_x3_upsample_phase_weights(const float* w, void* planes, int Cout, int C, float scale, void* stream);
 int ief_gemm_x3p_tile_bm(int tile);
 int ief_gemm_x3p_tile_bn(int tile);
```
